# NoahVl/Explaining-In-Style-Reproducibility-Study

Measured on AMD Instinct MI355X. Metric: StylEx G+D+enc train-step images/sec @256px, higher is better.
Workload: dtype bf16; 1 GPU; FFHQ-shaped 256x256 StylEx, batch 32/GPU, GAE=2 (noise+encoder micro-steps), GP every 4th step, ResNet-18 classifier; image_size=256, batch_per_gpu=32, start_step=0, gradient_accumulate_every=2, global_batch=32, parallelism=dp1

## Files before the change

### explaining-in-style-reproducibility-study_amd/csrc/conv_halo_dma.hip

```cpp
#include <hip/hip_runtime.h>
#include <stdint.h>
#include <stdlib.h>

#include <type_traits>

#include "stylex_internal.h"

typedef float f32x16 __attribute__((ext_vector_type(16)));
typedef short bf16x8 __attribute__((ext_vector_type(8)));
typedef __bf16 bf16x2_t __attribute__((ext_vector_type(2)));
typedef float f32x2_t __attribute__((ext_vector_type(2)));

namespace {

__device__ uint4 g_zero_page_fwd[4];

typedef __attribute__((address_space(3))) void* lds_void_ptr;
typedef __attribute__((address_space(1))) const void* gl_void_ptr;

__device__ __forceinline__ unsigned short to_bf16(float v) {
    f32x2_t t = {v, 0.f};
    bf16x2_t r = __builtin_convertvector(t, bf16x2_t);
    return (unsigned short)(*reinterpret_cast<unsigned*>(&r) & 0xffffu);
}

constexpr int TW = 32, TH = 16, HWD = TW + 2, NP = (TH + 2) * HWD;
constexpr int ROW = 32;
constexpr int HALO_PIECES = (NP + 31) / 32;
constexpr int HALO_BYTES = HALO_PIECES * 1024;
template <int TNJ>
struct DmaCfg {
    static constexpr int BN = TNJ * 32;
    static constexpr int W_PIECES = 9 * BN / 32;
    static constexpr int PIECES = HALO_PIECES + W_PIECES;
    static constexpr int NIT = (PIECES + 3) / 4;
    static constexpr int BUF = PIECES * 1024;
    static constexpr int SMEM_BYTES = 2 * BUF;
};

template <int TNJ, unsigned MASK>
__device__ __forceinline__ void dma_chunk_masked(const char* base, const int (&a_off)[6][3], int b_lane,
                                                 f32x16 (&acc)[4][TNJ]) {
    constexpr int BN = TNJ * 32;
#pragma unroll
    for (int tap = 0; tap < 9; ++tap) {
        if (!((MASK >> tap) & 1u)) continue;
        const int kh = tap / 3, kw = tap - kh * 3;
        const int slot = __builtin_popcount(MASK & ((1u << tap) - 1u));
        bf16x8 av[4], bv[TNJ];
#pragma unroll
        for (int i = 0; i < 4; ++i) av[i] = *reinterpret_cast<const bf16x8*>(base + a_off[i + kh][kw]);
#pragma unroll
        for (int j = 0; j < TNJ; ++j)
            bv[j] = *reinterpret_cast<const bf16x8*>(base + b_lane + (slot * BN + j * 32) * ROW);
#pragma unroll
        for (int i = 0; i < 4; ++i)
#pragma unroll
            for (int j = 0; j < TNJ; ++j)
                acc[i][j] = __builtin_amdgcn_mfma_f32_32x32x16_bf16(bv[j], av[i], acc[i][j], 0, 0, 0);
    }
}

constexpr unsigned S2D_DGRAD_MASK[4] = {1u << 4, (1u << 4) | (1u << 5), (1u << 4) | (1u << 7),
                                        (1u << 4) | (1u << 5) | (1u << 7) | (1u << 8)};

constexpr unsigned S2D_FWD_MASK[4] = {1u << 4, (1u << 3) | (1u << 4), (1u << 1) | (1u << 4),
                                      (1u << 0) | (1u << 1) | (1u << 3) | (1u << 4)};
__device__ __forceinline__ int s2d_fwd_taps(int q) { return q == 0 ? 0x4 : q == 1 ? 0x43 : q == 2 ? 0x41 : 0x4310; }
__device__ __forceinline__ int s2d_fwd_ntaps(int q) { return q == 0 ? 1 : q == 3 ? 4 : 2; }

template <int TNJ, bool S2D = false>
__global__ __launch_bounds__(256, TNJ == 4 ? 1 : 2) void conv3x3_halo_dma_kernel(ConvKParams p) {
    constexpr int BN = DmaCfg<TNJ>::BN, PIECES = DmaCfg<TNJ>::PIECES, NIT = DmaCfg<TNJ>::NIT, BUF = DmaCfg<TNJ>::BUF;
    extern __shared__ __attribute__((aligned(16))) char smem[];
    const int tid = threadIdx.x, lane = tid & 63, wave = tid >> 6;
    const int H = p.Ho, W = p.Wo, C = p.Ck, N = p.N;
    const int n_tiles = (N + BN - 1) / BN;
    const int tiles_x = (W + TW - 1) / TW, tiles_y = (H + TH - 1) / TH;

    int bid = blockIdx.x;
    {
        int nblk = gridDim.x, q = nblk >> 3, rr = nblk & 7, xcd = bid & 7, idx = bid >> 3;
        bid = (xcd < rr ? xcd * (q + 1) : rr * (q + 1) + (xcd - rr) * q) + idx;
    }
    const int n0 = (bid % n_tiles) * BN;
    int pt = bid / n_tiles;
    const int b = pt / (tiles_x * tiles_y);
    pt -= b * tiles_x * tiles_y;
    const int y0 = (pt / tiles_x) * TH, x0 = (pt % tiles_x) * TW;

    const unsigned short* xs = reinterpret_cast<const unsigned short*>(p.a);
    const unsigned short* ws = reinterpret_cast<const unsigned short*>(p.w);
    const unsigned short* zero = reinterpret_cast<const unsigned short*>(g_zero_page_fwd);
    const int lr = lane >> 1, pslot = lane & 1;
    const int slot = pslot ^ ((lr >> 3) & 1);

    long src_off[NIT];
    bool src_ok[NIT];
    int wslot[NIT];
#pragma unroll
    for (int it = 0; it < NIT; ++it) {
        const int piece = wave + 4 * it;
        src_off[it] = 0;
        src_ok[it] = false;
        wslot[it] = 0;
        if (piece >= PIECES) continue;
        if (piece < HALO_PIECES) {
            const int hp = piece * 32 + lr;
            const int hh = hp / HWD, ww = hp - hh * HWD;
            const int y = y0 - 1 + hh, x = x0 - 1 + ww;
            src_ok[it] = hp < NP && y >= 0 && y < H && x >= 0 && x < W;
            src_off[it] = ((long)(b * H + y) * W + x) * C + slot * 8;
        } else {
            const int r = (piece - HALO_PIECES) * 32 + lr;
            int tap = r / BN;
            const int nl = r - tap * BN;
            bool tap_ok = true;
            wslot[it] = tap;
            if (S2D && !p.flip_taps) {
                tap = 0;
            } else if (S2D) {
                const unsigned m = S2D_DGRAD_MASK[n0 / p.s2d_c];
                tap_ok = tap < __builtin_popcount(m);
                unsigned mm = m;
// ... 104 lines not shown
        const bool more = ch + 1 < nchunks;
        const char* base = smem + buf * BUF;
#pragma unroll
        for (int tap = 0; tap < 9; ++tap) {
            const int kh = tap / 3, kw = tap - kh * 3;
            bf16x8 av[4], bv[TNJ];
#pragma unroll
            for (int i = 0; i < 4; ++i)
                av[i] = *reinterpret_cast<const bf16x8*>(base + a_off[i + kh][kw]);
#pragma unroll
            for (int j = 0; j < TNJ; ++j)
                bv[j] = *reinterpret_cast<const bf16x8*>(base + b_lane + (tap * BN + j * 32) * ROW);
#pragma unroll
            for (int i = 0; i < 4; ++i)
#pragma unroll
                for (int j = 0; j < TNJ; ++j)
                    acc[i][j] = __builtin_amdgcn_mfma_f32_32x32x16_bf16(bv[j], av[i], acc[i][j], 0, 0, 0);
            if (more && 2 * tap < NIT) {
                issue_piece((ch + 1) * 16, buf ^ 1, 2 * tap);
                if (2 * tap + 1 < NIT) issue_piece((ch + 1) * 16, buf ^ 1, 2 * tap + 1);
            }
        }
    }
    const int lj = lane & 31, lh = lane >> 5;
    const bool act = (p.flags & (STYLEX_EPI_LRELU | STYLEX_EPI_RELU)) != 0;
    const float slope = (p.flags & STYLEX_EPI_RELU) ? 0.f : 0.2f;
    unsigned short* yout = reinterpret_cast<unsigned short*>(p.y);
    const unsigned short* gate = (!S2D && (p.flags & STYLEX_EPI_GATE)) ? reinterpret_cast<const unsigned short*>(p.residual) : nullptr;
    const float gslope = p.res_scale;
    const unsigned char* gmask = S2D ? nullptr : p.gate_mask;
    unsigned char* mask_out = S2D ? nullptr : p.mask;
    auto gatem = [&](unsigned u, unsigned bits) -> unsigned {
        const float a0 = __uint_as_float(u << 16), c0 = __uint_as_float(u & 0xffff0000u);
        return (unsigned)to_bf16((bits & 1u) ? a0 : gslope * a0) | ((unsigned)to_bf16((bits & 2u) ? c0 : gslope * c0) << 16);
    };
    auto gate2 = [&](unsigned u, unsigned g) -> unsigned {
        const float a0 = __uint_as_float(u << 16), c0 = __uint_as_float(u & 0xffff0000u);
        const float ga = __uint_as_float(g << 16), gc = __uint_as_float(g & 0xffff0000u);
        return (unsigned)to_bf16(ga > 0.f ? a0 : gslope * a0) | ((unsigned)to_bf16(gc > 0.f ? c0 : gslope * c0) << 16);
    };
    {
        const unsigned short* res = (S2D && (p.flags & STYLEX_EPI_RESIDUAL)) ? reinterpret_cast<const unsigned short*>(p.residual) : nullptr;
        const float rsc = p.res_scale;
        const bool merged = S2D && !p.flip_taps && p.x2 != nullptr;
        float4 b4[TNJ][4];
#pragma unroll
        for (int j = 0; j < TNJ; ++j)
#pragma unroll
            for (int g = 0; g < 4; ++g) {
                const int n = n0 + j * 32 + 8 * g + 4 * lh;
                b4[j][g] = ((p.flags & STYLEX_EPI_BIAS) && n < N) ? *reinterpret_cast<const float4*>(p.bias + n)
                                                                  : make_float4(0.f, 0.f, 0.f, 0.f);
            }
#pragma unroll
        for (int i = 0; i < 4; ++i) {
            const int y = y0 + 4 * wave + i, x = x0 + lj;
            const bool pix_ok = y < H && x < W;
            const long obase = ((long)(b * H + y) * W + x) * N;
#pragma unroll
            for (int j = 0; j < TNJ; ++j) {
                unsigned P[4][2];
#pragma unroll
                for (int g = 0; g < 4; ++g) {
                    float v0 = acc[i][j][4 * g + 0] + b4[j][g].x, v1 = acc[i][j][4 * g + 1] + b4[j][g].y;
                    float v2 = acc[i][j][4 * g + 2] + b4[j][g].z, v3 = acc[i][j][4 * g + 3] + b4[j][g].w;
                    if (res) {
                        const int n = n0 + j * 32 + 8 * g + 4 * lh;
                        uint2 rv = make_uint2(0u, 0u);
                        if (pix_ok && n < N) rv = *reinterpret_cast<const uint2*>(res + obase + n);
                        v0 = (v0 + __uint_as_float(rv.x << 16)) * rsc;
                        v1 = (v1 + __uint_as_float(rv.x & 0xffff0000u)) * rsc;
                        v2 = (v2 + __uint_as_float(rv.y << 16)) * rsc;
                        v3 = (v3 + __uint_as_float(rv.y & 0xffff0000u)) * rsc;
                    } else if (merged) {
                        v0 *= rsc;
                        v1 *= rsc;
                        v2 *= rsc;
                        v3 *= rsc;
                    }
                    if (act) {
                        v0 = v0 > 0.f ? v0 : slope * v0;
                        v1 = v1 > 0.f ? v1 : slope * v1;
                        v2 = v2 > 0.f ? v2 : slope * v2;
                        v3 = v3 > 0.f ? v3 : slope * v3;
                    }
                    P[g][0] = (unsigned)to_bf16(v0) | ((unsigned)to_bf16(v1) << 16);
                    P[g][1] = (unsigned)to_bf16(v2) | ((unsigned)to_bf16(v3) << 16);
                }
#pragma unroll
                for (int g = 0; g < 4; g += 2)
#pragma unroll
                    for (int h = 0; h < 2; ++h) {
                        auto r = __builtin_amdgcn_permlane32_swap(P[g][h], P[g + 1][h], false, false);
                        P[g][h] = r[0];
                        P[g + 1][h] = r[1];
                    }
#pragma unroll
                for (int q = 0; q < 2; ++q) {
                    const int n = n0 + j * 32 + 16 * q + 8 * lh;
                    if (pix_ok && n < N) {
                        uint4 v = make_uint4(P[2 * q][0], P[2 * q][1], P[2 * q + 1][0], P[2 * q + 1][1]);
                        const long o = obase + n;
                        if (gate) {
                            const uint4 gv = *reinterpret_cast<const uint4*>(gate + o);
                            v.x = gate2(v.x, gv.x);
                            v.y = gate2(v.y, gv.y);
                            v.z = gate2(v.z, gv.z);
                            v.w = gate2(v.w, gv.w);
                        } else if (gmask) {
                            const unsigned m = gmask[o >> 3];
                            v.x = gatem(v.x, m);
                            v.y = gatem(v.y, m >> 2);
                            v.z = gatem(v.z, m >> 4);
                            v.w = gatem(v.w, m >> 6);
                        }
                        *reinterpret_cast<uint4*>(yout + o) = v;
                        if (mask_out) mask_out[o >> 3] = (unsigned char)stylex_sign_bits8(v);
                    }
                }
            }
        }
    }
}

}

template <int TNJ, bool S2D = false>
static int launch_dma(const ConvKParams& p, hipStream_t s) {
    static bool attr_done = false;
    if (!attr_done) {
        hipError_t e = hipFuncSetAttribute(reinterpret_cast<const void*>(conv3x3_halo_dma_kernel<TNJ, S2D>),
                                           hipFuncAttributeMaxDynamicSharedMemorySize, DmaCfg<TNJ>::SMEM_BYTES);
        if (e != hipSuccess) return (int)e;
        attr_done = true;
    }
    long tiles = (long)p.B * ((p.Wo + TW - 1) / TW) * ((p.Ho + TH - 1) / TH);
    long blocks = tiles * ((p.N + DmaCfg<TNJ>::BN - 1) / DmaCfg<TNJ>::BN);
    stylex_note_kernel("conv3x3_halo_dma_kernel<%d, %s>", TNJ, S2D ? "true" : "false");
    hipLaunchKernelGGL((conv3x3_halo_dma_kernel<TNJ, S2D>), dim3((unsigned)blocks), dim3(256), DmaCfg<TNJ>::SMEM_BYTES, s, p);
    return (int)hipGetLastError();
}

int stylex_launch_halo_dma(const ConvKParams& p, hipStream_t s) {
    static const bool on = !(getenv("STYLEX_HALO_DMA") && getenv("STYLEX_HALO_DMA")[0] == '0');
    static const bool on64 = !(getenv("STYLEX_HALO_DMA64") && getenv("STYLEX_HALO_DMA64")[0] == '0');
    static const bool on_s2d = !(getenv("STYLEX_HALO_DMA_S2D") && getenv("STYLEX_HALO_DMA_S2D")[0] == '0');
    if (!on) return STYLEX_NOT_APPLICABLE;
    if (!p.act_bf16 || p.a_scale) return STYLEX_NOT_APPLICABLE;
    if (p.flags & ~(STYLEX_EPI_BIAS | STYLEX_EPI_LRELU | STYLEX_EPI_RELU |
                    (p.s2d_c ? STYLEX_EPI_RESIDUAL : (STYLEX_EPI_GATE | STYLEX_EPI_GATE_MASK | STYLEX_EPI_MASK_OUT))))
        return STYLEX_NOT_APPLICABLE;
    if (p.s2d_c && (p.mask || p.gate_mask)) return STYLEX_NOT_APPLICABLE;
    if (p.x2) {
        if (!p.s2d_c || p.flip_taps || !p.w2 || p.c2 < 8 || p.c2 % 8 != 0 || (p.flags & STYLEX_EPI_RESIDUAL)) return STYLEX_NOT_APPLICABLE;
        if ((reinterpret_cast<uintptr_t>(p.x2) & 15) || (reinterpret_cast<uintptr_t>(p.w2) & 15)) return STYLEX_NOT_APPLICABLE;
    }
    if ((p.flags & STYLEX_EPI_GATE) && (!p.residual || (reinterpret_cast<uintptr_t>(p.residual) & 15))) return STYLEX_NOT_APPLICABLE;
    if (p.s2d_c && on_s2d) {
        const int rc = p.flip_taps ? stylex_launch_s2d_dgrad(p, s) : stylex_launch_s2d_fwd(p, s);
        if (rc != STYLEX_NOT_APPLICABLE) return rc;
    }
    if (p.N % 8 != 0 || p.Ck % 8 != 0 || p.Wo < 32 || p.Ho < 16) return STYLEX_NOT_APPLICABLE;
    if ((reinterpret_cast<uintptr_t>(p.a) & 15) || (reinterpret_cast<uintptr_t>(p.w) & 15) ||
        (reinterpret_cast<uintptr_t>(p.y) & 15))
        return STYLEX_NOT_APPLICABLE;
    if (p.s2d_c) {
        if (!on_s2d || !on64 || p.s2d_c % 64 != 0) return STYLEX_NOT_APPLICABLE;
        if (p.flip_taps) {
            if (p.flags || p.N != 4 * p.s2d_c || p.Ck < 64) return STYLEX_NOT_APPLICABLE;
        } else {
            static const bool on_fwd = !(getenv("STYLEX_HALO_DMA_S2D_FWD") && getenv("STYLEX_HALO_DMA_S2D_FWD")[0] == '0');
            if (!on_fwd || (p.flags & ~(STYLEX_EPI_BIAS | STYLEX_EPI_RESIDUAL)) || p.Ck != 4 * p.s2d_c || p.N % 64 != 0)
                return STYLEX_NOT_APPLICABLE;
            if ((p.flags & STYLEX_EPI_RESIDUAL) && (!p.residual || (reinterpret_cast<uintptr_t>(p.residual) & 15)))
                return STYLEX_NOT_APPLICABLE;
        }
        return p.dry ? 0 : launch_dma<2, true>(p, s);
    }
    if (on64 && p.Ck >= 64 && p.N % 64 == 0) return p.dry ? 0 : launch_dma<2>(p, s);
    static const bool on32 = !(getenv("STYLEX_HALO_DMA32") && getenv("STYLEX_HALO_DMA32")[0] == '0');
    if (on32 && on64 && p.Ck >= 64 && p.N <= 32) return p.dry ? 0 : launch_dma<1>(p, s);
    if (p.N >= 128 && p.Ck >= 128) return p.dry ? 0 : launch_dma<4>(p, s);
    return STYLEX_NOT_APPLICABLE;
}
```

### explaining-in-style-reproducibility-study_amd/csrc/conv_pipe.hip

```cpp
#include <hip/hip_runtime.h>
#include <stdint.h>
#include <stdlib.h>

#include "stylex_internal.h"

#ifndef PIPE_STORE_AUX
#define PIPE_STORE_AUX 0
#endif

typedef float f32x16 __attribute__((ext_vector_type(16)));
typedef short bf16x8 __attribute__((ext_vector_type(8)));
typedef __bf16 bf16x2_t __attribute__((ext_vector_type(2)));
typedef float f32x2_t __attribute__((ext_vector_type(2)));
typedef unsigned u32x4 __attribute__((ext_vector_type(4)));

struct StylexPipeArgs {
    int total_tiles;
    unsigned m_ntiles, m_tpi, m_tx;
    int dbg;
};

#ifdef STYLEX_PIPE_ABLATION
#define PIPE_DBG (pa.dbg)
#else
#define PIPE_DBG 0
#endif


namespace {

typedef StylexPipeArgs PipeArgs;
typedef __attribute__((address_space(3))) void* lds_void_ptr;

__device__ __forceinline__ unsigned short to_bf16(float v) {
    f32x2_t t = {v, 0.f};
    bf16x2_t r = __builtin_convertvector(t, bf16x2_t);
    return (unsigned short)(*reinterpret_cast<unsigned*>(&r) & 0xffffu);
}

template <int NT>
struct PipeCfg {
    static constexpr int TH = NT == 128 ? 16 : 32;
    static constexpr int TW = 32, HWD = TW + 2, NP = (TH + 2) * HWD;
    static constexpr int H_PIECES = (NP + 31) / 32;
    static constexpr int H_STRIDE = H_PIECES * 1024;
    static constexpr int W_PIECES = 9 * NT / 32;
    static constexpr int W_STRIDE = W_PIECES * 1024;
    static constexpr int HS = 3, WS = 2;
    static constexpr int W_BASE = HS * H_STRIDE;
    static constexpr int BIAS_BASE = W_BASE + WS * W_STRIDE;
    static constexpr int DUMP_BASE = BIAS_BASE + 2048;
    static constexpr int SMEM = DUMP_BASE + 1024;
    static constexpr int HP_MAX = (H_PIECES + 7) / 8;
    static constexpr int WP_MAX = (W_PIECES + 7) / 8;
    static constexpr int RG = TH / 4;
};

__device__ __forceinline__ void dma16(__amdgpu_buffer_rsrc_t r, char* smem, int lds_off, unsigned voff, unsigned soff) {
    __builtin_amdgcn_raw_ptr_buffer_load_lds(r, (lds_void_ptr)(smem + lds_off), 16, voff, soff, 0, 0);
}

template <int N>
__device__ __forceinline__ void wait_vmcnt() {
    asm volatile("s_waitcnt vmcnt(%0)" ::"n"(N) : "memory");
}

template <int OFF>
__device__ __forceinline__ void lds_read16(bf16x8& dst, int addr) {
    asm volatile("ds_read_b128 %0, %1 offset:%2" : "=v"(dst) : "v"(addr), "n"(OFF));
}
__device__ __forceinline__ void lds_wait(bf16x8 (&av)[4], bf16x8 (&bv)[2]) {
    asm volatile("s_waitcnt lgkmcnt(0)" : "+v"(av[0]), "+v"(av[1]), "+v"(av[2]), "+v"(av[3]), "+v"(bv[0]), "+v"(bv[1]));
}
template <int HWD, int TAP>
__device__ __forceinline__ void tap_addr(int (&addr)[4], int a_base, unsigned& swz) {
    constexpr int kh = TAP / 3, kw = TAP % 3;
    asm volatile("" : "+v"(swz));
#pragma unroll
    for (int i = 0; i < 4; ++i) addr[i] = a_base + ((i + kh) * HWD + kw) * 32 + (int)(((swz >> ((i + kh) * 3 + kw)) & 1u) << 4);
}
template <int NT, int TAP>
__device__ __forceinline__ void load_tap(bf16x8 (&av)[4], bf16x8 (&bv)[2], const int (&addr)[4], int b_addr) {
    lds_read16<(TAP * NT) * 32>(bv[0], b_addr);
    lds_read16<(TAP * NT + 32) * 32>(bv[1], b_addr);
#pragma unroll
    for (int i = 0; i < 4; ++i) lds_read16<0>(av[i], addr[i]);
}

__device__ __forceinline__ void mfma1(f32x16& acc, const bf16x8& a, const bf16x8& b) {
    asm volatile("v_mfma_f32_32x32x16_bf16 %0, %1, %2, %0" : "+v"(acc) : "v"(a), "v"(b));
}
__device__ __forceinline__ void mfma8(f32x16 (&acc)[4][2], const bf16x8 (&av)[4], const bf16x8 (&bv)[2]) {
#pragma unroll
    for (int i = 0; i < 4; ++i)
#pragma unroll
        for (int j = 0; j < 2; ++j) mfma1(acc[i][j], bv[j], av[i]);
}

__device__ __forceinline__ int fastdiv(int n, unsigned magic) { return magic ? (int)__umulhi((unsigned)n, magic) : n; }


template <int NT, int EPI>
__global__ __launch_bounds__(512, 2) void conv3x3_pipe_kernel(ConvKParams p, PipeArgs pa) {
    using Cfg = PipeCfg<NT>;
    constexpr int TH = Cfg::TH, HWD = Cfg::HWD, NP = Cfg::NP, H_PIECES = Cfg::H_PIECES, H_STRIDE = Cfg::H_STRIDE;
// ... 74 lines not shown
#pragma unroll
    for (int r = 0; r < 6; ++r)
#pragma unroll
        for (int kw = 0; kw < 3; ++kw) {
            const int t = a_row + r * HWD + kw;
            swz |= (unsigned)(((t >> 3) ^ lk) & 1) << (r * 3 + kw);
        }
    const int b_cur0 = W_BASE + (nh * 64 + li) * 32 + ((((li >> 3) ^ lk) & 1) << 4), b_cur1 = b_cur0 + W_STRIDE;

    if (EPI == 0 && (p.flags & STYLEX_EPI_BIAS) && tid < N) reinterpret_cast<float*>(smem + Cfg::BIAS_BASE)[tid] = p.bias[tid];

    f32x16 acc[4][2];
    auto zero_acc = [&]() {
#pragma unroll
        for (int i = 0; i < 4; ++i)
#pragma unroll
            for (int j = 0; j < 2; ++j)
#pragma unroll
                for (int e = 0; e < 16; ++e) acc[i][j][e] = 0.f;
    };
    zero_acc();

    const bool act = EPI == 0 && (p.flags & (STYLEX_EPI_LRELU | STYLEX_EPI_RELU)) != 0;
    const float slope = (p.flags & STYLEX_EPI_RELU) ? 0.f : 0.2f;
    const float gslope = p.res_scale;
    const bool mask_out = EPI == 0 && p.mask != nullptr;
    auto gatem = [&](unsigned u, unsigned bits) -> unsigned {
        const float a0 = __uint_as_float(u << 16), c0 = __uint_as_float(u & 0xffff0000u);
        f32x2_t t = {(bits & 1u) ? a0 : gslope * a0, (bits & 2u) ? c0 : gslope * c0};
        bf16x2_t r = __builtin_convertvector(t, bf16x2_t);
        return *reinterpret_cast<unsigned*>(&r);
    };
    auto gate2 = [&](unsigned u, unsigned g) -> unsigned {
        const float a0 = __uint_as_float(u << 16), c0 = __uint_as_float(u & 0xffff0000u);
        const float ga = __uint_as_float(g << 16), gc = __uint_as_float(g & 0xffff0000u);
        f32x2_t t = {ga > 0.f ? a0 : gslope * a0, gc > 0.f ? c0 : gslope * c0};
        bf16x2_t r = __builtin_convertvector(t, bf16x2_t);
        return *reinterpret_cast<unsigned*>(&r);
    };
    const unsigned bytes_y = (unsigned)((long)p.B * H * W * N * 2);
    const __amdgpu_buffer_rsrc_t ry = __builtin_amdgcn_make_buffer_rsrc(p.y, 0, (int)bytes_y, 0x00020000);
    const __amdgpu_buffer_rsrc_t rgate = __builtin_amdgcn_make_buffer_rsrc(const_cast<float*>(p.residual), 0, (int)bytes_y, 0x00020000);
    const __amdgpu_buffer_rsrc_t rmask = __builtin_amdgcn_make_buffer_rsrc(
        EPI == 2 ? const_cast<unsigned char*>(p.gate_mask) : p.mask, 0, (int)(bytes_y >> 4), 0x00020000);
    const unsigned rowb = (unsigned)(W * N) * 2u;
    auto pack2 = [](float a, float c) -> unsigned {
        f32x2_t t = {a, c};
        bf16x2_t r = __builtin_convertvector(t, bf16x2_t);
        return *reinterpret_cast<unsigned*>(&r);
    };
    const unsigned lane_off = (unsigned)(((4 * rg) * W + (lane & 7)) * N + nh * 64) * 2u +
                              (unsigned)(4 * ((lane >> 4) & 1) + 2 * ((lane >> 3) & 1) + (lane >> 5)) * 16u;
    const unsigned pixb8 = (unsigned)N * 16u;
    auto epilogue = [&](int b, int y0, int x0, int n0) {
        const int lh = lk;
        const int nb = n0 + nh * 64;
        const unsigned t_off = __builtin_amdgcn_readfirstlane((unsigned)((((long)(b * H + y0) * W + x0) * N + n0) * 2));
        const unsigned g_off = x0 + li < W ? (unsigned)(((4 * rg) * W + li) * N + nh * 64 + 8 * lh) * 2u : OOB;
#pragma unroll
        for (int i = 0; i < 4; ++i) {
            const bool row_ok = y0 + 4 * rg + i < H;
            const unsigned soff = t_off + i * rowb;
            u32x4 R[4];
#pragma unroll
            for (int j = 0; j < 2; ++j) {
                u32x4 gv[2];
                unsigned gm[2];
                if (EPI != 0) {
                    const unsigned voff = row_ok ? g_off : OOB;
#pragma unroll
                    for (int q = 0; q < 2; ++q) {
                        if (EPI == 1) gv[q] = __builtin_amdgcn_raw_buffer_load_b128(rgate, voff + (j * 64 + q * 32), soff, 0);
                        if (EPI == 2) gm[q] = __builtin_amdgcn_raw_buffer_load_b8(rmask, (voff >> 4) + (j * 4 + q * 2), soff >> 4, 0);
                    }
                }
                float4 b4[4];
#pragma unroll
                for (int g = 0; g < 4; ++g)
                    b4[g] = (EPI == 0 && (p.flags & STYLEX_EPI_BIAS))
                                ? *reinterpret_cast<const float4*>(smem + Cfg::BIAS_BASE + (nb + j * 32 + 8 * g + 4 * lh) * 4)
                                : make_float4(0.f, 0.f, 0.f, 0.f);
                unsigned P[4][2];
#pragma unroll
                for (int g = 0; g < 4; ++g) {
                    float v0 = acc[i][j][4 * g + 0] + b4[g].x, v1 = acc[i][j][4 * g + 1] + b4[g].y;
                    float v2 = acc[i][j][4 * g + 2] + b4[g].z, v3 = acc[i][j][4 * g + 3] + b4[g].w;
                    if (act) {
                        v0 = v0 > 0.f ? v0 : slope * v0;
                        v1 = v1 > 0.f ? v1 : slope * v1;
                        v2 = v2 > 0.f ? v2 : slope * v2;
                        v3 = v3 > 0.f ? v3 : slope * v3;
                    }
                    P[g][0] = pack2(v0, v1);
                    P[g][1] = pack2(v2, v3);
                }
#pragma unroll
                for (int g = 0; g < 4; g += 2)
#pragma unroll
                    for (int h = 0; h < 2; ++h) {
                        auto r = __builtin_amdgcn_permlane32_swap(P[g][h], P[g + 1][h], false, false);
                        P[g][h] = r[0];
                        P[g + 1][h] = r[1];
                    }
#pragma unroll
                for (int q = 0; q < 2; ++q) {
                    uint4 v = make_uint4(P[2 * q][0], P[2 * q][1], P[2 * q + 1][0], P[2 * q + 1][1]);
                    if (EPI == 1) {
                        v.x = gate2(v.x, gv[q].x);
                        v.y = gate2(v.y, gv[q].y);
                        v.z = gate2(v.z, gv[q].z);
                        v.w = gate2(v.w, gv[q].w);
                    } else if (EPI == 2) {
                        const unsigned m = gm[q];
                        v.x = gatem(v.x, m);
                        v.y = gatem(v.y, m >> 2);
                        v.z = gatem(v.z, m >> 4);
// ... 113 lines not shown
    __builtin_amdgcn_sched_barrier(0);
#define PIPE_CHUNK(A1, B1, A2, B2, BCUR, BNEXT, MORE_W, MORE_H)                                    \
    {                                                                                              \
        const bool mw_ = MORE_W, mh_ = MORE_H;                                                     \
        const unsigned w_soff = (unsigned)(w_n0 * 9 * C + w_ch * 16) * 2u, h_soff = (unsigned)h_ch * 32u; \
        PIPE_TAP(0, A1, B1, A2, B2, BCUR, mw_, mh_)                                                \
        PIPE_TAP(1, A2, B2, A1, B1, BCUR, mw_, mh_)                                                \
        PIPE_TAP(2, A1, B1, A2, B2, BCUR, mw_, mh_)                                                \
        PIPE_TAP(3, A2, B2, A1, B1, BCUR, mw_, mh_)                                                \
        PIPE_TAP(4, A1, B1, A2, B2, BCUR, mw_, mh_)                                                \
        PIPE_TAP(5, A2, B2, A1, B1, BCUR, mw_, mh_)                                                \
        PIPE_TAP(6, A1, B1, A2, B2, BCUR, mw_, mh_)                                                \
        PIPE_TAP(7, A2, B2, A1, B1, BCUR, mw_, mh_)                                                \
        PIPE_LAST(A1, B1, A2, B2, BNEXT)                                                           \
        if (mw_) adv_w();                                                                          \
        if (mh_) adv_h();                                                                          \
    }
    for (int g = 0; g < total; g += 2) {
        PIPE_CHUNK(avA, bvA, avB, bvB, b_cur0, b_cur1, g + 1 < total, g + 2 < total)
        PIPE_CHUNK(avB, bvB, avA, bvA, b_cur1, b_cur0, g + 2 < total, g + 3 < total)
        c_ch += 2;
        if (c_ch == nchunks) {
            c_ch = 0;
            asm volatile("s_nop 15\n\ts_nop 15"
                         : "+v"(acc[0][0]), "+v"(acc[0][1]), "+v"(acc[1][0]), "+v"(acc[1][1]), "+v"(acc[2][0]), "+v"(acc[2][1]),
                           "+v"(acc[3][0]), "+v"(acc[3][1]));
            epilogue(cb, cy0, cx0, cn0);
            if (++c_k < my_tiles) {
                decode(c_k, cb, cy0, cx0, cn0);
                zero_acc();
            }
        }
    }
#undef PIPE_CHUNK
#undef PIPE_LAST
#undef PIPE_TAP
#undef PIPE_DMA
#undef issue_h1
#undef issue_w1
    asm volatile("s_waitcnt lgkmcnt(0)" ::: "memory");
    wait_vmcnt<0>();
}

int g_num_cus = 0;

unsigned magic_of(int d) { return d <= 1 ? 0u : (unsigned)(((1ull << 32) + (unsigned)d - 1) / (unsigned)d); }

template <int NT, int EPI>
int launch_pipe(const ConvKParams& p, hipStream_t s) {
    using Cfg = PipeCfg<NT>;
    static bool attr_done = false;
    if (!attr_done) {
        hipError_t e = hipFuncSetAttribute(reinterpret_cast<const void*>(conv3x3_pipe_kernel<NT, EPI>),
                                           hipFuncAttributeMaxDynamicSharedMemorySize, Cfg::SMEM);
        if (e != hipSuccess) return (int)e;
        attr_done = true;
    }
    if (!g_num_cus) {
        int dev = 0, n = 0;
        (void)hipGetDevice(&dev);
        (void)hipDeviceGetAttribute(&n, hipDeviceAttributeMultiprocessorCount, dev);
        g_num_cus = n > 0 ? (n & ~7) : 256;
        if (g_num_cus < 8) g_num_cus = 8;
    }
    const int tiles_x = (p.Wo + 31) / 32, tiles_y = (p.Ho + Cfg::TH - 1) / Cfg::TH, n_tiles = p.N / NT;
    PipeArgs pa;
    pa.total_tiles = p.B * tiles_x * tiles_y * n_tiles;
    pa.m_ntiles = magic_of(n_tiles);
    pa.m_tpi = magic_of(tiles_x * tiles_y);
    pa.m_tx = magic_of(tiles_x);
#ifdef STYLEX_PIPE_ABLATION
    pa.dbg = getenv("STYLEX_PIPE_DBG") ? atoi(getenv("STYLEX_PIPE_DBG")) : 0;
#else
    pa.dbg = 0;
#endif
    stylex_note_kernel("conv3x3_pipe_kernel<%d, %d>", NT, EPI);
    hipLaunchKernelGGL((conv3x3_pipe_kernel<NT, EPI>), dim3((unsigned)g_num_cus), dim3(512), Cfg::SMEM, s, p, pa);
    return (int)hipGetLastError();
}

template <int NT>
int launch_pipe_epi(const ConvKParams& p, hipStream_t s) {
    if (p.flags & STYLEX_EPI_GATE) return launch_pipe<NT, 1>(p, s);
    if (p.flags & STYLEX_EPI_GATE_MASK) return launch_pipe<NT, 2>(p, s);
    return launch_pipe<NT, 0>(p, s);
}

}

int stylex_launch_pipe(const ConvKParams& p, hipStream_t s) {
    const char* env = getenv("STYLEX_CONV_PIPE");
    if (env && env[0] == '0') return STYLEX_NOT_APPLICABLE;
    if (!p.act_bf16 || p.a_scale || p.s2d_c) return STYLEX_NOT_APPLICABLE;
    if (p.flags & ~(STYLEX_EPI_BIAS | STYLEX_EPI_LRELU | STYLEX_EPI_RELU | STYLEX_EPI_GATE | STYLEX_EPI_GATE_MASK | STYLEX_EPI_MASK_OUT))
        return STYLEX_NOT_APPLICABLE;
    if ((p.flags & STYLEX_EPI_GATE) && (!p.residual || (reinterpret_cast<uintptr_t>(p.residual) & 15))) return STYLEX_NOT_APPLICABLE;
    if (p.Ck < 64 || p.Ck % 32 != 0 || p.N % 64 != 0 || p.N > 512 || p.Wo < 32 || p.Ho < 16) return STYLEX_NOT_APPLICABLE;
    if ((reinterpret_cast<uintptr_t>(p.a) & 15) || (reinterpret_cast<uintptr_t>(p.w) & 15) || (reinterpret_cast<uintptr_t>(p.y) & 15))
        return STYLEX_NOT_APPLICABLE;
    if ((long)p.B * p.Ho * p.Wo * p.Ck * 2 >= (1l << 31) || (long)p.N * 9 * p.Ck * 2 >= (1l << 31) ||
        (long)p.B * p.Ho * p.Wo * p.N * 2 >= (1l << 31))
        return STYLEX_NOT_APPLICABLE;
    const bool n128 = p.N % 128 == 0 && !(env && env[0] == '6');
    if (!n128) {
        if (p.Ho < 32 && !(env && env[0] == '6')) return STYLEX_NOT_APPLICABLE;
        if (!(env && env[0] == '6') && ((p.flags & STYLEX_EPI_GATE) || (p.flip_taps && !p.flags && p.Ck == 64)))
            return STYLEX_NOT_APPLICABLE;
    }
    if (p.dry) return 0;
    if (n128) return launch_pipe_epi<128>(p, s);
    return launch_pipe_epi<64>(p, s);
}
```

### explaining-in-style-reproducibility-study_amd/csrc/elementwise.hip

```cpp
#include <hip/hip_runtime.h>
#include <stdint.h>

#include "stylex_internal.h"

namespace {

template <int V>
struct Vec;
template <>
struct Vec<4> {
    typedef float4 T;
    static __device__ __forceinline__ T zero() { return make_float4(0.f, 0.f, 0.f, 0.f); }
    static __device__ __forceinline__ T ld(const void* p, long off, int bf) { return act_ld4(p, off, bf); }
    static __device__ __forceinline__ void st(void* p, long off, T v, int bf) { act_st4(p, off, v, bf); }
    static __device__ __forceinline__ void fma(T& a, float w, T x) {
        a.x = fmaf(w, x.x, a.x); a.y = fmaf(w, x.y, a.y); a.z = fmaf(w, x.z, a.z); a.w = fmaf(w, x.w, a.w);
    }
};
template <>
struct Vec<1> {
    typedef float T;
    static __device__ __forceinline__ T zero() { return 0.f; }
    static __device__ __forceinline__ T ld(const void* p, long off, int bf) { return act_ld1(p, off, bf); }
    static __device__ __forceinline__ void st(void* p, long off, T v, int bf) { act_st1(p, off, v, bf); }
    static __device__ __forceinline__ void fma(T& a, float w, T x) { a = fmaf(w, x, a); }
};

struct F8 {
    float4 a, b;
};
template <>
struct Vec<8> {
    typedef F8 T;
    static __device__ __forceinline__ T zero() { return F8{make_float4(0.f, 0.f, 0.f, 0.f), make_float4(0.f, 0.f, 0.f, 0.f)}; }
    static __device__ __forceinline__ T ld(const void* p, long off, int) {
        uint4 h = *reinterpret_cast<const uint4*>(reinterpret_cast<const unsigned short*>(p) + off);
        return F8{act_unpack4(make_uint2(h.x, h.y)), act_unpack4(make_uint2(h.z, h.w))};
    }
    static __device__ __forceinline__ void st(void* p, long off, T v, int) {
        uint2 lo = act_pack4(v.a), hi = act_pack4(v.b);
        *reinterpret_cast<uint4*>(reinterpret_cast<unsigned short*>(p) + off) = make_uint4(lo.x, lo.y, hi.x, hi.y);
    }
    static __device__ __forceinline__ void fma(T& acc, float w, T x) {
        Vec<4>::fma(acc.a, w, x.a);
        Vec<4>::fma(acc.b, w, x.b);
    }
};

__device__ __forceinline__ void up_rule(int o, int n, int& lo, int& hi, float& w_hi) {
    int k = o >> 1;
    if (o & 1) {
        lo = k;
        hi = min(k + 1, n - 1);
        w_hi = 0.25f;
    } else {
        lo = max(k - 1, 0);
        hi = k;
        w_hi = 0.75f;
    }
}
__device__ __forceinline__ float up_coef(int o, int i, int n) {
    int lo, hi;
    float wh;
    up_rule(o, n, lo, hi, wh);
    return (lo == i ? 1.f - wh : 0.f) + (hi == i ? wh : 0.f);
}

__device__ __forceinline__ long decomp_index(long i, int cv, int Wd, int Hd, int& cq, int& w, int& h, int& b) {
    if (i < (1L << 31)) {
        const unsigned u = (unsigned)i, pix = u / (unsigned)cv, r = pix / (unsigned)Wd;
        cq = (int)(u - pix * (unsigned)cv);
        w = (int)(pix - r * (unsigned)Wd);
        b = (int)(r / (unsigned)Hd);
        h = (int)(r - (unsigned)b * (unsigned)Hd);
        return (long)pix;
    }
    const long pix = i / cv, r = pix / Wd;
    cq = (int)(i - pix * cv);
    w = (int)(pix - r * Wd);
    b = (int)(r / Hd);
    h = (int)(r - (long)b * Hd);
    return pix;
}

template <int V>
__global__ void upsample2x_fwd_kernel(const void* __restrict__ x, void* __restrict__ y, int B, int H, int W, int C, int bf) {
    const int cv = C / V;
    const long total = (long)B * 2 * H * 2 * W * cv;
    for (long i = blockIdx.x * (long)blockDim.x + threadIdx.x; i < total; i += (long)gridDim.x * blockDim.x) {
        int cq, ow, oh, b;
        const long pix = decomp_index(i, cv, (2 * W), (2 * H), cq, ow, oh, b);
        const int c = cq * V;
        int hl, hh, wl, wh_;
        float fh, fw;
        up_rule(oh, H, hl, hh, fh);
        up_rule(ow, W, wl, wh_, fw);
        const long base = (long)b * H * W * C + c;
        typename Vec<V>::T acc = Vec<V>::zero();
        typename Vec<V>::T r0 = Vec<V>::zero(), r1 = Vec<V>::zero();
        Vec<V>::fma(r0, 1.f - fw, Vec<V>::ld(x, base + ((long)hl * W + wl) * C, bf));
        Vec<V>::fma(r0, fw, Vec<V>::ld(x, base + ((long)hl * W + wh_) * C, bf));
        Vec<V>::fma(r1, 1.f - fw, Vec<V>::ld(x, base + ((long)hh * W + wl) * C, bf));
        Vec<V>::fma(r1, fw, Vec<V>::ld(x, base + ((long)hh * W + wh_) * C, bf));
        Vec<V>::fma(acc, 1.f - fh, r0);
        Vec<V>::fma(acc, fh, r1);
        Vec<V>::st(y, pix * C + c, acc, bf);
    }
}

template <int V>
__global__ void upsample2x_bwd_kernel(const void* __restrict__ dy, void* __restrict__ dx, int B, int H, int W, int C, int bf) {
    const int cv = C / V;
    const long total = (long)B * H * W * cv;
    for (long i = blockIdx.x * (long)blockDim.x + threadIdx.x; i < total; i += (long)gridDim.x * blockDim.x) {
        int cq, iw, ih, b;
        const long pix = decomp_index(i, cv, W, H, cq, iw, ih, b);
        const int c = cq * V;
        const long base = (long)b * 4 * H * W * C + c;
        typename Vec<V>::T acc = Vec<V>::zero();
#pragma unroll
        for (int a = -1; a <= 2; ++a) {
            int oh = 2 * ih + a;
            if (oh < 0 || oh >= 2 * H) continue;
            float ch = up_coef(oh, ih, H);
            if (ch == 0.f) continue;
#pragma unroll
            for (int e = -1; e <= 2; ++e) {
                int ow = 2 * iw + e;
                if (ow < 0 || ow >= 2 * W) continue;
                float cw = up_coef(ow, iw, W);
                if (cw == 0.f) continue;
                Vec<V>::fma(acc, ch * cw, Vec<V>::ld(dy, base + ((long)oh * 2 * W + ow) * C, bf));
            }
        }
        Vec<V>::st(dx, pix * C + c, acc, bf);
    }
}

__device__ __forceinline__ int reflect1(int i, int n) { return i < 0 ? -i : (i >= n ? 2 * n - 2 - i : i); }

__device__ __forceinline__ float ub_coef(int o, int i, int n) {
    const int n2 = 2 * n;
    return 0.25f * up_coef(reflect1(o - 1, n2), i, n) + 0.5f * up_coef(o, i, n) + 0.25f * up_coef(reflect1(o + 1, n2), i, n);
}

template <int V>
__global__ void rgb_up_blur_add_fwd_kernel(const void* __restrict__ rgb, const void* __restrict__ prev, void* __restrict__ y,
                                           int B, int H, int W, int C, int bf) {
    const int cv = C / V;
    const long total = (long)B * 2 * H * 2 * W * cv;
    for (long i = blockIdx.x * (long)blockDim.x + threadIdx.x; i < total; i += (long)gridDim.x * blockDim.x) {
        int cq, ow, oh, b;
        const long pix = decomp_index(i, cv, 2 * W, 2 * H, cq, ow, oh, b);
        const int c = cq * V, kh = oh >> 1, kw = ow >> 1;
        const long base = (long)b * H * W * C + c;
        float cw[3];
#pragma unroll
        for (int e = 0; e < 3; ++e) {
            const int iw = kw - 1 + e;
            cw[e] = (iw >= 0 && iw < W) ? ub_coef(ow, iw, W) : 0.f;
        }
        typename Vec<V>::T acc = Vec<V>::zero();
// ... 326 lines not shown
    long b = (work + 255) / 256;
    if (b > 2048) b = 2048;
    if (b < 1) b = 1;
    return (int)b;
}
inline bool vec_ok(int C, const void* a, const void* b) {
    return (C % 4 == 0) && ((reinterpret_cast<uintptr_t>(a) & 15) == 0) && ((reinterpret_cast<uintptr_t>(b) & 15) == 0);
}

}

#define LAUNCH_EW(kern, work, a, b, ...)                                                                    \
    do {                                                                                                    \
        if (bf && (C % 8 == 0) && vec_ok(C, a, b))                                                          \
            hipLaunchKernelGGL(kern<8>, dim3(grid_for((work) / 8)), dim3(256), 0, s, __VA_ARGS__);          \
        else if (vec_ok(C, a, b))                                                                           \
            hipLaunchKernelGGL(kern<4>, dim3(grid_for((work) / 4)), dim3(256), 0, s, __VA_ARGS__);          \
        else                                                                                                \
            hipLaunchKernelGGL(kern<1>, dim3(grid_for(work)), dim3(256), 0, s, __VA_ARGS__);                \
        return (int)hipGetLastError();                                                                      \
    } while (0)

static bool blur_strip_ok(int bf, int H, int C, const void* a, const void* b) {
    return bf && (C % 8 == 0) && H >= 8 && ((reinterpret_cast<uintptr_t>(a) & 15) == 0) &&
           ((reinterpret_cast<uintptr_t>(b) & 15) == 0);
}
template <bool ADJ>
static int launch_blur_strip(const void* in, void* out, int B, int H, int W, int C, int s2d, hipStream_t s,
                             const void* gate = nullptr, float gslope = 0.f, const void* gmask = nullptr) {
    constexpr int ROWS = 8;
    long work = (long)B * ((H + ROWS - 1) / ROWS) * W * (C / 8);
    long blocks = (work + 255) / 256;
    if (blocks > 16384) blocks = 16384;
    hipLaunchKernelGGL((blur3x3_strip_kernel<ADJ, ROWS>), dim3((unsigned)blocks), dim3(256), 0, s,
                       (const unsigned short*)in, (unsigned short*)out, B, H, W, C, s2d, (const unsigned short*)gate,
                       gslope, (const unsigned char*)gmask);
    return (int)hipGetLastError();
}

extern "C" {

#define EW_ARGS const int64_t* sh, int act_dtype, void* stream
#define EW_UNPACK                                                     \
    hipStream_t s = (hipStream_t)stream;                               \
    int B = (int)sh[0], H = (int)sh[1], W = (int)sh[2], C = (int)sh[3]; \
    int bf = act_dtype == 1;                                           \
    if (act_dtype != 0 && act_dtype != 1) return STYLEX_EINVAL;

int stylex_upsample2x_bilinear_fwd(const void* x, void* y, EW_ARGS) {
    EW_UNPACK
    if (B <= 0 || H <= 0 || W <= 0 || C <= 0) return STYLEX_EINVAL;
    LAUNCH_EW(upsample2x_fwd_kernel, (long)B * 4 * H * W * C, x, y, x, y, B, H, W, C, bf);
}
int stylex_upsample2x_bilinear_bwd(const void* dy, void* dx, EW_ARGS) {
    EW_UNPACK
    if (B <= 0 || H <= 0 || W <= 0 || C <= 0) return STYLEX_EINVAL;
    LAUNCH_EW(upsample2x_bwd_kernel, (long)B * H * W * C, dy, dx, dy, dx, B, H, W, C, bf);
}
int stylex_rgb_up_blur_add_fwd(const void* rgb, const void* prev, void* y, EW_ARGS) {
    EW_UNPACK
    if (!rgb || !y || B <= 0 || H <= 0 || W <= 0 || C <= 0) return STYLEX_EINVAL;
    const void* al = prev ? prev : rgb;
    if (vec_ok(C, rgb, y) && vec_ok(C, al, y))
        hipLaunchKernelGGL(rgb_up_blur_add_fwd_kernel<4>, dim3(grid_for((long)B * 4 * H * W * C / 4)), dim3(256), 0, s, rgb, prev,
                           y, B, H, W, C, bf);
    else
        hipLaunchKernelGGL(rgb_up_blur_add_fwd_kernel<1>, dim3(grid_for((long)B * 4 * H * W * C)), dim3(256), 0, s, rgb, prev, y,
                           B, H, W, C, bf);
    return (int)hipGetLastError();
}
int stylex_rgb_up_blur_add_bwd(const void* dy, void* dx, EW_ARGS) {
    EW_UNPACK
    if (!dy || !dx || B <= 0 || H <= 0 || W <= 0 || C <= 0) return STYLEX_EINVAL;
    LAUNCH_EW(rgb_up_blur_add_bwd_kernel, (long)B * H * W * C, dy, dx, dy, dx, B, H, W, C, bf);
}
int stylex_blur3x3_reflect_fwd(const void* x, void* y, EW_ARGS) {
    EW_UNPACK
    if (B <= 0 || H < 2 || W < 2 || C <= 0) return STYLEX_EINVAL;
    if (blur_strip_ok(bf, H, C, x, y)) return launch_blur_strip<false>(x, y, B, H, W, C, 0, s);
    LAUNCH_EW(blur3x3_fwd_kernel, (long)B * H * W * C, x, y, x, y, B, H, W, C, bf, 0);
}
static int blur_bwd_impl(const void* dy, const void* gate, float gslope, void* dx, int s2d, EW_ARGS) {
    EW_UNPACK
    if (B <= 0 || H < 2 || W < 2 || C <= 0 || (s2d && ((H & 1) || (W & 1)))) return STYLEX_EINVAL;
    const bool gate_ok = !gate || (reinterpret_cast<uintptr_t>(gate) & 15) == 0;
    if (gate_ok && blur_strip_ok(bf, H, C, dy, dx)) return launch_blur_strip<true>(dy, dx, B, H, W, C, s2d, s, gate, gslope);
    if (gate && !gate_ok) {
        hipLaunchKernelGGL(blur3x3_bwd_kernel<1>, dim3(grid_for((long)B * H * W * C)), dim3(256), 0, s, dy, dx, B, H, W, C, bf,
                           s2d, gate, gslope);
        return (int)hipGetLastError();
    }
    LAUNCH_EW(blur3x3_bwd_kernel, (long)B * H * W * C, dy, dx, dy, dx, B, H, W, C, bf, s2d, gate, gslope);
}
int stylex_blur3x3_reflect_bwd(const void* dy, void* dx, EW_ARGS) { return blur_bwd_impl(dy, nullptr, 0.f, dx, 0, sh, act_dtype, stream); }
int stylex_blur3x3_reflect_bwd_gate(const void* dy, const void* gate, float slope, void* dx, EW_ARGS) {
    if (!gate) return STYLEX_EINVAL;
    return blur_bwd_impl(dy, gate, slope, dx, 0, sh, act_dtype, stream);
}
int stylex_blur3x3_s2d_bwd_gate(const void* dy, const void* gate, float slope, void* dx, EW_ARGS) {
    if (!gate) return STYLEX_EINVAL;
    return blur_bwd_impl(dy, gate, slope, dx, 1, sh, act_dtype, stream);
}
int stylex_blur3x3_s2d_bwd_gate_mask(const void* dy, const void* mask, float slope, void* dx, EW_ARGS) {
    EW_UNPACK
    if (!dy || !mask || !dx || B <= 0 || H < 2 || W < 2 || C <= 0 || (H & 1) || (W & 1)) return STYLEX_EINVAL;
    if (!blur_strip_ok(bf, H, C, dy, dx)) return STYLEX_EINVAL;
// ... 82 lines not shown
```

### explaining-in-style-reproducibility-study_amd/csrc/fused_bwd.hip

```cpp
#include <hip/hip_runtime.h>
#include <stdint.h>

#include "stylex_internal.h"

namespace {

constexpr int NT = 256;

template <int K>
struct Acc {
    float4 v[K];
    __device__ __forceinline__ void zero() {
#pragma unroll
        for (int k = 0; k < K; ++k) v[k] = make_float4(0.f, 0.f, 0.f, 0.f);
    }
};

template <int K>
__device__ __forceinline__ void block_reduce_store(Acc<K>& a, float* smem, int cv, int prow, int CV, int rpp, int C,
                                                   float* partial_row , bool active) {
    float4* s4 = reinterpret_cast<float4*>(smem);
    if (active) {
#pragma unroll
        for (int k = 0; k < K; ++k) s4[(k * rpp + prow) * CV + cv] = a.v[k];
// ... 100 lines not shown
            float4 yv = ld4(y, o, bf);
            float nz = 0.f;
            if (noise) {
                const int pi = (int)p, h = pi / W, w = pi - h * W;
                nz = noise[((long)g.b * ns + w) * ns + h];
            }
            float4 t = yv;
            if (lrelu) {
                gv.x = yv.x > 0.f ? gv.x : 0.2f * gv.x; t.x = yv.x > 0.f ? yv.x : 5.f * yv.x;
                gv.y = yv.y > 0.f ? gv.y : 0.2f * gv.y; t.y = yv.y > 0.f ? yv.y : 5.f * yv.y;
                gv.z = yv.z > 0.f ? gv.z : 0.2f * gv.z; t.z = yv.z > 0.f ? yv.z : 5.f * yv.z;
                gv.w = yv.w > 0.f ? gv.w : 0.2f * gv.w; t.w = yv.w > 0.f ? yv.w : 5.f * yv.w;
            }
            if (gz_scale) st4(gz, o, make_float4(gv.x * d4.x, gv.y * d4.y, gv.z * d4.z, gv.w * d4.w), bf);
            else st4(gz, o, gv, bf);
            a.v[0].x += gv.x * (t.x - (nz * w4.x + b4.x));
            a.v[0].y += gv.y * (t.y - (nz * w4.y + b4.y));
            a.v[0].z += gv.z * (t.z - (nz * w4.z + b4.z));
            a.v[0].w += gv.w * (t.w - (nz * w4.w + b4.w));
            a.v[1].x += gv.x * nz; a.v[1].y += gv.y * nz; a.v[1].z += gv.z * nz; a.v[1].w += gv.w * nz;
            a.v[2].x += gv.x; a.v[2].y += gv.y; a.v[2].z += gv.z; a.v[2].w += gv.w;
        }
    }
    block_reduce_store<3>(a, smem, g.cv, g.prow, g.CV, g.rpp, C, partial + ((long)g.b * nchunks + blockIdx.x) * 3 * C,
                          g.active && c < C);
}

__global__ __launch_bounds__(NT) void scale_reduce_kernel(const void* __restrict__ x, const void* __restrict__ t,
                                                         const float* __restrict__ s, void* __restrict__ gx,
                                                         float* __restrict__ partial, int HW, int C, int nchunks, int bf) {
    extern __shared__ __attribute__((aligned(16))) float smem[];
    Geo g = make_geo(HW, C, nchunks);
    Acc<1> a;
    a.zero();
    const int c = g.cv * 4;
    if (g.active && c < C) {
        float4 s4 = ldp4(s + (long)g.b * C + c);
        const long base = (long)g.b * HW;
        for (long p = g.p_begin + g.prow; p < g.p_end; p += g.rpp) {
            const long o = (base + p) * C + c;
            float4 tv = ld4(t, o, bf);
            float4 xv = ld4(x, o, bf);
            a.v[0].x += xv.x * tv.x; a.v[0].y += xv.y * tv.y; a.v[0].z += xv.z * tv.z; a.v[0].w += xv.w * tv.w;
            if (gx) {
                tv.x *= s4.x; tv.y *= s4.y; tv.z *= s4.z; tv.w *= s4.w;
                st4(gx, o, tv, bf);
            }
        }
    }
    block_reduce_store<1>(a, smem, g.cv, g.prow, g.CV, g.rpp, C, partial + ((long)g.b * nchunks + blockIdx.x) * C,
                          g.active && c < C);
}

inline size_t reduce_smem(int C, int K) {
    int CV = (C + 3) / 4;
    if (CV > NT) CV = NT;
    int rpp = NT / CV;
    return (size_t)K * rpp * CV * 16;
}

inline bool ok_shape(const int64_t* sh, int nchunks) {
    return sh[0] > 0 && sh[1] > 0 && sh[2] > 0 && sh[3] > 0 && sh[3] <= 1024 && (sh[3] % 4 == 0) && nchunks > 0 &&
           sh[0] <= 65535;
}

}

extern "C" {

int stylex_reduce_chunks(const int64_t* sh) {
    long HW = (long)sh[1] * sh[2];
    long n = (2048 + sh[0] - 1) / sh[0];
    long maxc = (HW + 63) / 64;
    if (n > maxc) n = maxc;
    if (n < 1) n = 1;
    return (int)n;
}

int stylex_act_bwd_reduce(const void* dy, const void* y, void* dx, float* partial, const int64_t* sh, int nchunks,
                          int lrelu, float scale, int act_dtype, void* stream) {
    if (act_dtype != 0 && act_dtype != 1) return STYLEX_EINVAL;
    if (!dy || !partial || !ok_shape(sh, nchunks) || (lrelu && !y)) return STYLEX_EINVAL;
    int HW = (int)(sh[1] * sh[2]), C = (int)sh[3];
    hipLaunchKernelGGL(act_bwd_reduce_kernel, dim3(nchunks, (unsigned)sh[0]), dim3(NT), reduce_smem(C, 1),
                       (hipStream_t)stream, dy, y, dx, partial, HW, C, nchunks, lrelu, scale, act_dtype);
    return (int)hipGetLastError();
}

static int modconv_bwd_prep_impl(const void* gy, const void* y, const float* noise, int64_t noise_stride,
                                 const float* noise_w, const float* noise_b, void* gz, float* partial, const int64_t* sh,
                                 int nchunks, int lrelu, int act_dtype, const float* gz_scale, void* stream);

int stylex_modconv_bwd_prep(const void* gy, const void* y, const float* noise, int64_t noise_stride,
                            const float* noise_w, const float* noise_b, void* gz, float* partial, const int64_t* sh,
                            int nchunks, int lrelu, int act_dtype, void* stream) {
    return modconv_bwd_prep_impl(gy, y, noise, noise_stride, noise_w, noise_b, gz, partial, sh, nchunks, lrelu, act_dtype,
                                 nullptr, stream);
}

int stylex_modconv_bwd_prep_scaled(const void* gy, const void* y, const float* noise, int64_t noise_stride,
                                   const float* noise_w, const float* noise_b, const float* gz_scale, void* gz,
                                   float* partial, const int64_t* sh, int nchunks, int lrelu, int act_dtype, void* stream) {
    if (!gz_scale || (reinterpret_cast<uintptr_t>(gz_scale) & 15)) return STYLEX_EINVAL;
    return modconv_bwd_prep_impl(gy, y, noise, noise_stride, noise_w, noise_b, gz, partial, sh, nchunks, lrelu, act_dtype,
                                 gz_scale, stream);
}

static int modconv_bwd_prep_impl(const void* gy, const void* y, const float* noise, int64_t noise_stride,
                                 const float* noise_w, const float* noise_b, void* gz, float* partial, const int64_t* sh,
                                 int nchunks, int lrelu, int act_dtype, const float* gz_scale, void* stream) {
    if (act_dtype != 0 && act_dtype != 1) return STYLEX_EINVAL;
    if (!gy || !y || !gz || !partial || !ok_shape(sh, nchunks)) return STYLEX_EINVAL;
    if (noise && (!noise_w || !noise_b || noise_stride < sh[1] || noise_stride < sh[2])) return STYLEX_EINVAL;
    int C = (int)sh[3];
    hipLaunchKernelGGL(modconv_bwd_prep_kernel, dim3(nchunks, (unsigned)sh[0]), dim3(NT), reduce_smem(C, 3),
                       (hipStream_t)stream, gy, y, noise, (int)noise_stride, noise_w, noise_b, gz, partial, (int)sh[1],
                       (int)sh[2], C, nchunks, lrelu, act_dtype, gz_scale);
    return (int)hipGetLastError();
}

int stylex_scale_reduce(const void* x, const void* t, const float* s, void* gx, float* partial, const int64_t* sh,
                        int nchunks, int act_dtype, void* stream) {
    if (act_dtype != 0 && act_dtype != 1) return STYLEX_EINVAL;
    if (!x || !t || !s || !partial || !ok_shape(sh, nchunks)) return STYLEX_EINVAL;
    int HW = (int)(sh[1] * sh[2]), C = (int)sh[3];
    hipLaunchKernelGGL(scale_reduce_kernel, dim3(nchunks, (unsigned)sh[0]), dim3(NT), reduce_smem(C, 1),
                       (hipStream_t)stream, x, t, s, gx, partial, HW, C, nchunks, act_dtype);
    return (int)hipGetLastError();
}

}
```

### explaining-in-style-reproducibility-study_amd/csrc/stylex_capi.hip

```cpp
#include <hip/hip_runtime.h>
#include <stdint.h>
#include <stdarg.h>
#include <stdio.h>
#include <string.h>

#include <array>
#include <map>
#include <mutex>
#include <string>
#include <vector>

#include "stylex_internal.h"

namespace {

typedef std::array<int64_t, 9> LayerKey;
struct TimedLaunch {
    hipEvent_t start, stop;
    int cls;
    double flops;
    double bytes;
    LayerKey key;
    char kernel[112];
};
// ... 202 lines not shown
static void bwd_data_params(ConvKParams& p, const int64_t* sh) {
    fill_common(p, sh);
    p.Hi = (int)sh[9];
    p.Wi = (int)sh[10];
    p.Ck = (int)sh[4];
    p.N = (int)sh[3];
    p.Ho = (int)sh[1];
    p.Wo = (int)sh[2];
    p.M = p.B * p.Ho * p.Wo;
}

int64_t stylex_conv2d_workspace_bytes(const int64_t* sh, int which, int precision) {
    if (!conv_shape_ok(sh) || (which != 0 && which != 1)) return STYLEX_EINVAL;
    ConvKParams p;
    if (which == 0) fwd_params(p, sh);
    else {
        bwd_data_params(p, sh);
        p.transposed = 1;
    }
    p.act_bf16 = precision == STYLEX_BF16_ACT;
    return stylex_igemm_workspace_bytes(p, precision);
}

int stylex_conv_mask_supported(const int64_t* sh, int which, int flags, int precision) {
    if (!conv_shape_ok(sh) || precision != STYLEX_BF16_ACT || (which != 0 && which != 1)) return 0;
    static const uintptr_t fake = 4096;
    ConvKParams p;
    if (which == 0) {
        if (!(flags & STYLEX_EPI_MASK_OUT) || !(flags & STYLEX_EPI_LRELU)) return 0;
        fwd_params(p, sh);
        if (p.N % 8 != 0) return 0;
        p.mask = (unsigned char*)fake;
    } else {
        if (!(flags & STYLEX_EPI_GATE_MASK) || (flags & ~(STYLEX_EPI_GATE_MASK))) return 0;
        bwd_data_params(p, sh);
        if (p.KH != 3 || p.stride != 1 || p.pad != 1) return 0;
        p.flip_taps = 1;
        p.gate_mask = (const unsigned char*)fake;
    }
    p.a = (const float*)fake;
    p.w = (const void*)fake;
    p.y = (float*)fake;
    p.bias = (const float*)fake;
    p.flags = flags;
    p.act_bf16 = 1;
    p.dry = 1;
    if (which == 0 && stylex_launch_rgb(p, nullptr) == 0) return 1;
    return stylex_launch_halo(p, nullptr) == 0 ? 1 : 0;
}

int stylex_conv2d_fwd(const void* x, const void* w_fwd, void* y, const int64_t* sh, int flags,
                      const stylex_conv_epilogue* epi, int precision, void* workspace, int64_t workspace_bytes,
                      void* stream) {
    if (!x || !w_fwd || !y || !conv_shape_ok(sh)) return STYLEX_EINVAL;
    if (precision != STYLEX_F32 && precision != STYLEX_BF16 && precision != STYLEX_BF16_ACT) return STYLEX_EINVAL;
    ConvKParams p;
    fwd_params(p, sh);
    p.a = (const float*)x;
    p.w = w_fwd;
    p.y = (float*)y;
    p.flags = flags;
    p.act_bf16 = precision == STYLEX_BF16_ACT;
    if (p.act_bf16) precision = STYLEX_BF16;
    if (epi) {
        p.a_scale = epi->in_scale;
        p.bias = epi->bias;
        p.out_scale = epi->out_scale;
        p.noise = epi->noise;
        p.noise_stride = (int)epi->noise_stride;
        p.noise_w = epi->noise_w;
        p.noise_b = epi->noise_b;
        p.residual = (const float*)epi->residual;
        p.res_scale = epi->res_scale;
        p.s2d_c = (int)epi->s2d_c;
    }
    if (flags & STYLEX_EPI_GATE_MASK) return STYLEX_EINVAL;
    if (flags & STYLEX_EPI_MASK_OUT) {
        if (!epi || !epi->mask || !(flags & STYLEX_EPI_LRELU) || !p.act_bf16 || p.N % 8 != 0) return STYLEX_EINVAL;
        p.mask = (unsigned char*)epi->mask;
    }
    if ((flags & STYLEX_EPI_BIAS) && !p.bias) return STYLEX_EINVAL;
    if ((flags & STYLEX_EPI_OSCALE) && !p.out_scale) return STYLEX_EINVAL;
    if ((flags & STYLEX_EPI_NOISE_NAT) && (!(flags & STYLEX_EPI_NOISE) || (reinterpret_cast<uintptr_t>(p.noise) & 15) ||
                                           p.noise_stride % 4 != 0))
        return STYLEX_EINVAL;
    if ((flags & STYLEX_EPI_NOISE) && (!p.noise || !p.noise_w || !p.noise_b || p.noise_stride < p.Ho || p.noise_stride < p.Wo))
        return STYLEX_EINVAL;
    if ((flags & STYLEX_EPI_RESIDUAL) && !p.residual) return STYLEX_EINVAL;
    if (p.s2d_c && (p.Ck != 4 * p.s2d_c || p.KH != 3 || p.stride != 1 || p.pad != 1 || p.s2d_c % 64)) return STYLEX_EINVAL;
    double flops = 2.0 * p.M * (double)p.N * p.Ck * p.KH * p.KW / (p.s2d_c ? 4.0 : 1.0);
    ScopedTimer tm(0, flops, conv_bytes(sh, p.act_bf16 ? STYLEX_BF16_ACT : precision, false), (hipStream_t)stream, sh, p.s2d_c);
    return stylex_launch_igemm(p, precision, workspace, workspace_bytes, (hipStream_t)stream);
}

static int s2d_res_params(ConvKParams& p, const int64_t* sh, int64_t s2d_c, int64_t res_c) {
    if (!conv_shape_ok(sh)) return STYLEX_EINVAL;
    fwd_params(p, sh);
    p.s2d_c = (int)s2d_c;
    p.c2 = (int)res_c;
    if (s2d_c <= 0 || s2d_c % 64 || p.Ck != 4 * p.s2d_c || p.KH != 3 || p.stride != 1 || p.pad != 1) return STYLEX_EINVAL;
    if (res_c < 8 || res_c % 8) return STYLEX_EINVAL;
    p.act_bf16 = 1;
    p.flags = STYLEX_EPI_BIAS;
    return 0;
}

int stylex_conv2d_s2d_res_supported(const int64_t* sh, int64_t s2d_c, int64_t res_c) {
    static const uintptr_t fake = 4096;
    ConvKParams p;
    if (s2d_res_params(p, sh, s2d_c, res_c)) return 0;
    p.a = (const float*)fake;
    p.w = (const void*)fake;
    p.y = (float*)fake;
    p.bias = (const float*)fake;
    p.x2 = p.w2 = (const void*)fake;
    p.dry = 1;
    return stylex_launch_halo_dma(p, nullptr) == 0 ? 1 : 0;
}

int stylex_conv2d_s2d_res_fwd(const void* x_s2d, const void* w_fwd_s2d, const void* x_res, const void* w_res, const float* bias,
                              void* y, const int64_t* sh, int64_t s2d_c, int64_t res_c, float scale, void* stream) {
    if (!x_s2d || !w_fwd_s2d || !x_res || !w_res || !bias || !y) return STYLEX_EINVAL;
    ConvKParams p;
    if (int rc = s2d_res_params(p, sh, s2d_c, res_c)) return rc;
    p.a = (const float*)x_s2d;
    p.w = w_fwd_s2d;
    p.y = (float*)y;
    p.bias = bias;
    p.x2 = x_res;
    p.w2 = w_res;
    p.res_scale = scale;
    const double flops = 2.0 * p.M * (double)p.N * (p.Ck * 9 / 4.0 + p.c2);
    ScopedTimer tm(0, flops, conv_bytes(sh, STYLEX_BF16_ACT, false) + 2.0 * p.M * p.c2, (hipStream_t)stream, sh, p.s2d_c);
    const int rc = stylex_launch_halo_dma(p, (hipStream_t)stream);
    return rc == STYLEX_NOT_APPLICABLE ? STYLEX_EINVAL : rc;
}

int stylex_conv2d_bwd_data(const void* dy, const void* w_bwd, void* dx, const int64_t* sh, int flags,
                           const stylex_conv_epilogue* epi, int precision, void* workspace, int64_t workspace_bytes,
                           void* stream) {
    if (!dy || !w_bwd || !dx || !conv_shape_ok(sh) || sh[7] > 2) return STYLEX_EINVAL;
    if (precision != STYLEX_F32 && precision != STYLEX_BF16 && precision != STYLEX_BF16_ACT) return STYLEX_EINVAL;
    if (flags & ~(STYLEX_EPI_OSCALE | STYLEX_EPI_GATE | STYLEX_EPI_GATE_MASK)) return STYLEX_EINVAL;
    if ((flags & STYLEX_EPI_GATE) && (!epi || !epi->residual)) return STYLEX_EINVAL;
// ... 173 lines not shown
```

### explaining-in-style-reproducibility-study_amd/csrc/stylex_internal.h

```cpp
#pragma once
#include <hip/hip_runtime.h>
#include <stdint.h>

#include "../../include/stylex_hip.h"
#include "act_io.h"

struct ConvKParams {
    const float* a;
    const float* a_scale;
    const void* w;
    const float* a2;
    const float* a2_scale;
    float* y;
    const float* bias;
    const float* out_scale;
    const float* noise;
    const float* noise_w;
    const float* noise_b;
    const float* residual;
    float res_scale;
    int noise_stride;
    int B, Hi, Wi, Ck, N, KH, KW, Ho, Wo, stride, pad;
    int transposed;
    int phase_major;
    int act_bf16;
    int s2d_c;
    int flip_taps;
    int M;
    int flags;
    long split_len;
    int ksplit;
    int kt_per_split;
    float* partial;
    unsigned char* mask;
    const unsigned char* gate_mask;
    int dry;
    float* bias_partial;
    const void* x2;
    const void* w2;
    int c2;
    float wg_scale;
    int wg_accumulate;
};

int stylex_launch_igemm(ConvKParams p, int precision, void* workspace, int64_t workspace_bytes, hipStream_t s);
int64_t stylex_igemm_workspace_bytes(const ConvKParams& p, int precision);
void stylex_wgrad_plan(const ConvKParams& p, int* tn, int* tc, int* splits, long* split_len);
int stylex_launch_wgrad(ConvKParams p, float* partial, float* dw_oihw, int precision, hipStream_t s, float* db = nullptr,
                        int* db_done = nullptr);
int stylex_launch_pack(const float* w, void* wf, void* wb, int N, int C, int T, int dtype, hipStream_t s);

#define STYLEX_NOT_APPLICABLE (-100)

void stylex_note_kernel(const char* fmt, ...);

#ifdef __HIPCC__
__device__ __forceinline__ unsigned stylex_sign_bits8(uint4 v) {
    const unsigned w[4] = {v.x, v.y, v.z, v.w};
    unsigned m = 0;
#pragma unroll
    for (int d = 0; d < 4; ++d) {
        m |= (__uint_as_float(w[d] << 16) > 0.f ? 1u : 0u) << (2 * d);
        m |= (__uint_as_float(w[d] & 0xffff0000u) > 0.f ? 1u : 0u) << (2 * d + 1);
    }
    return m;
}
#endif
int stylex_launch_halo(const ConvKParams& p, hipStream_t s);

int stylex_launch_halo_dma(const ConvKParams& p, hipStream_t s);

int stylex_launch_rgb(const ConvKParams& p, hipStream_t s);

int stylex_launch_pipe(const ConvKParams& p, hipStream_t s);
int stylex_launch_line64(const ConvKParams& p, hipStream_t s);

int stylex_launch_s2d_dgrad(const ConvKParams& p, hipStream_t s);
int stylex_launch_s2d_fwd(const ConvKParams& p, hipStream_t s);

int stylex_launch_gather(ConvKParams& p, void* workspace, int64_t workspace_bytes, hipStream_t s);
int64_t stylex_gather_workspace_bytes(const ConvKParams& p);

bool stylex_wgrad_pipe_applicable(const ConvKParams& p);
void stylex_wgrad_pipe_plan(const ConvKParams& p, int* slices, int* tiles_per_split, int* blocks);
int stylex_launch_wgrad_pipe(ConvKParams p, float* partial, hipStream_t s, int* slices_out, int* bias_done = nullptr);
int stylex_launch_wgrad_s2d_folded(ConvKParams p, float* partial, float* dw_oihw, hipStream_t s);

bool stylex_wgrad_tr_applicable(const ConvKParams& p);
void stylex_wgrad_tr_plan(const ConvKParams& p, int* mode, int* splits, long* split_len);
int stylex_launch_wgrad_tr(ConvKParams p, float* partial, hipStream_t s, int* splits_out);

__host__ __device__ inline unsigned stylex_s2d_tap_mask(int s) {
    const int sy = s >> 1, sx = s & 1;
    unsigned m = 0;
    for (int kh = 0; kh < 2; ++kh)
        for (int kw = 0; kw < 2; ++kw)
            if ((kh == 1 || sy == 1) && (kw == 1 || sx == 1)) m |= 1u << (kh * 3 + kw);
    return m;
}
int stylex_launch_pack_s2d(const float* w, void* wf, void* wb, int N, int C, hipStream_t s);
int stylex_launch_fold_s2d(const float* dw2, float* dw, int N, int C, hipStream_t s);
```

### explaining-in-style-reproducibility-study_amd/stylex/hip_backend.py

```python
import os as _os

if _os.environ.get("STYLEX_MIOPEN_ALLOW_BWD_GTC", "0") != "1":
    _os.environ.setdefault("MIOPEN_DEBUG_CONV_IMPLICIT_GEMM_ASM_BWD_GTC_XDLOPS_NHWC", "0")

import atexit
import ctypes
import os
import weakref

import torch

_HERE = os.path.dirname(os.path.abspath(__file__))
LIB_PATH = os.path.join(os.path.dirname(_HERE), "libstylex_hip.so")

F32, BF16, BF16_ACT = 0, 1, 2
EPI_BIAS, EPI_LRELU, EPI_OSCALE, EPI_NOISE, EPI_RESIDUAL, EPI_RELU, EPI_GATE, EPI_NOISE_NAT = 1, 2, 4, 8, 16, 32, 64, 128
EPI_MASK_OUT, EPI_GATE_MASK = 256, 512

_c_f = ctypes.c_void_p
_i64p = ctypes.POINTER(ctypes.c_int64)


class ConvEpilogue(ctypes.Structure):
    _fields_ = [
        ("in_scale", ctypes.c_void_p),
        ("bias", ctypes.c_void_p),
        ("out_scale", ctypes.c_void_p),
        ("noise", ctypes.c_void_p),
        ("noise_stride", ctypes.c_int64),
        ("noise_w", ctypes.c_void_p),
        ("noise_b", ctypes.c_void_p),
        ("residual", ctypes.c_void_p),
        ("res_scale", ctypes.c_float),
        ("s2d_c", ctypes.c_int32),
        ("mask", ctypes.c_void_p),
    ]


SIGNATURES = {
    "stylex_init": (ctypes.c_int, [ctypes.c_int]),
    "stylex_version": (ctypes.c_char_p, []),
    "stylex_pack_weight": (ctypes.c_int, [_c_f, _c_f, _c_f, _i64p, ctypes.c_int, ctypes.c_void_p]),
    "stylex_conv2d_workspace_bytes": (ctypes.c_int64, [_i64p, ctypes.c_int, ctypes.c_int]),
    "stylex_conv2d_fwd": (ctypes.c_int, [_c_f, _c_f, _c_f, _i64p, ctypes.c_int, ctypes.POINTER(ConvEpilogue),
                                         ctypes.c_int, ctypes.c_void_p, ctypes.c_int64, ctypes.c_void_p]),
    "stylex_conv2d_bwd_data": (ctypes.c_int, [_c_f, _c_f, _c_f, _i64p, ctypes.c_int, ctypes.POINTER(ConvEpilogue),
                                              ctypes.c_int, ctypes.c_void_p, ctypes.c_int64, ctypes.c_void_p]),
    "stylex_conv2d_bwd_weight_workspace_bytes": (ctypes.c_int64, [_i64p]),
    "stylex_conv2d_bwd_weight": (ctypes.c_int, [_c_f, _c_f, _c_f, ctypes.c_void_p, ctypes.c_int64, _i64p, _c_f, _c_f,
                                                ctypes.c_int, ctypes.c_int, ctypes.c_void_p]),
    "stylex_conv2d_bwd_weight_bias": (ctypes.c_int, [_c_f, _c_f, _c_f, _c_f, ctypes.POINTER(ctypes.c_int), ctypes.c_void_p,
                                                     ctypes.c_int64, _i64p, _c_f, _c_f, ctypes.c_int, ctypes.c_int,
                                                     ctypes.c_void_p]),
    "stylex_conv2d_bwd_weight_ex": (ctypes.c_int, [_c_f, _c_f, _c_f, _c_f, ctypes.POINTER(ctypes.c_int), ctypes.c_void_p,
                                                   ctypes.c_int64, _i64p, _c_f, _c_f, ctypes.c_int, ctypes.c_float, ctypes.c_int,
                                                   ctypes.c_int, ctypes.c_void_p]),
    "stylex_blur3x3_s2d_fwd": (ctypes.c_int, [_c_f, _c_f, _i64p, ctypes.c_int, ctypes.c_void_p]),
    "stylex_blur3x3_s2d_bwd": (ctypes.c_int, [_c_f, _c_f, _i64p, ctypes.c_int, ctypes.c_void_p]),
    "stylex_blur3x3_reflect_bwd_gate": (ctypes.c_int, [_c_f, _c_f, ctypes.c_float, _c_f, _i64p, ctypes.c_int, ctypes.c_void_p]),
    "stylex_blur3x3_s2d_bwd_gate": (ctypes.c_int, [_c_f, _c_f, ctypes.c_float, _c_f, _i64p, ctypes.c_int, ctypes.c_void_p]),
    "stylex_blur3x3_s2d_bwd_gate_mask": (ctypes.c_int, [_c_f, _c_f, ctypes.c_float, _c_f, _i64p, ctypes.c_int, ctypes.c_void_p]),
    "stylex_conv_mask_supported": (ctypes.c_int, [_i64p, ctypes.c_int, ctypes.c_int, ctypes.c_int]),
    "stylex_add_at_even": (ctypes.c_int, [_c_f, _c_f, _i64p, ctypes.c_int, ctypes.c_void_p]),
    "stylex_subsample2_fwd": (ctypes.c_int, [_c_f, _c_f, _i64p, ctypes.c_int, ctypes.c_void_p]),
    "stylex_subsample2_bwd": (ctypes.c_int, [_c_f, _c_f, _i64p, ctypes.c_int, ctypes.c_void_p]),
    "stylex_pack_weight_s2d": (ctypes.c_int, [_c_f, _c_f, _c_f, _i64p, ctypes.c_void_p]),
    "stylex_fold_weight_grad_s2d": (ctypes.c_int, [_c_f, _c_f, _i64p, ctypes.c_void_p]),
    "stylex_conv2d_bwd_weight_s2d_supported": (ctypes.c_int, [_i64p, ctypes.c_int, ctypes.c_int]),
    "stylex_conv2d_bwd_weight_s2d": (ctypes.c_int, [ctypes.c_void_p, ctypes.c_void_p, _c_f, ctypes.c_void_p, ctypes.c_int64, _i64p,
                                                    ctypes.c_int, ctypes.c_float, ctypes.c_int, ctypes.c_int, ctypes.c_void_p]),
    "stylex_upsample2x_bilinear_fwd": (ctypes.c_int, [_c_f, _c_f, _i64p, ctypes.c_int, ctypes.c_void_p]),
    "stylex_upsample2x_bilinear_bwd": (ctypes.c_int, [_c_f, _c_f, _i64p, ctypes.c_int, ctypes.c_void_p]),
    "stylex_rgb_up_blur_add_fwd": (ctypes.c_int, [_c_f, _c_f, _c_f, _i64p, ctypes.c_int, ctypes.c_void_p]),
    "stylex_rgb_up_blur_add_bwd": (ctypes.c_int, [_c_f, _c_f, _i64p, ctypes.c_int, ctypes.c_void_p]),
    "stylex_blur3x3_reflect_fwd": (ctypes.c_int, [_c_f, _c_f, _i64p, ctypes.c_int, ctypes.c_void_p]),
    "stylex_blur3x3_reflect_bwd": (ctypes.c_int, [_c_f, _c_f, _i64p, ctypes.c_int, ctypes.c_void_p]),
    "stylex_bias_act_fwd": (ctypes.c_int, [_c_f, _c_f, _c_f, ctypes.c_int64, _c_f, _c_f, _c_f, _i64p, ctypes.c_int,
                                           ctypes.c_void_p]),
    "stylex_bias_act_bwd": (ctypes.c_int, [_c_f, _c_f, _c_f, _i64p, ctypes.c_int, ctypes.c_void_p]),
    "stylex_rowwise_sumsq": (ctypes.c_int, [_c_f, _c_f, _i64p, ctypes.c_void_p]),
    "stylex_reduce_chunks": (ctypes.c_int, [_i64p]),
    "stylex_act_bwd_reduce": (ctypes.c_int, [_c_f, _c_f, _c_f, _c_f, _i64p, ctypes.c_int, ctypes.c_int, ctypes.c_float,
                                             ctypes.c_int, ctypes.c_void_p]),
    "stylex_modconv_bwd_prep": (ctypes.c_int, [_c_f, _c_f, _c_f, ctypes.c_int64, _c_f, _c_f, _c_f, _c_f, _i64p,
                                               ctypes.c_int, ctypes.c_int, ctypes.c_int, ctypes.c_void_p]),
    "stylex_modconv_bwd_prep_scaled": (ctypes.c_int, [_c_f, _c_f, _c_f, ctypes.c_int64, _c_f, _c_f, _c_f, _c_f, _c_f, _i64p,
                                                      ctypes.c_int, ctypes.c_int, ctypes.c_int, ctypes.c_void_p]),
    "stylex_scale_reduce": (ctypes.c_int, [_c_f, _c_f, _c_f, _c_f, _c_f, _i64p, ctypes.c_int, ctypes.c_int,
                                           ctypes.c_void_p]),
    "stylex_pad_rgb8": (ctypes.c_int, [_c_f, _c_f, _i64p, _i64p, ctypes.c_int, ctypes.c_void_p]),
    "stylex_affine_act_nchw_fwd": (ctypes.c_int, [_c_f, _c_f, _c_f, _c_f, _c_f, ctypes.c_int64, ctypes.c_int64, ctypes.c_int64,
                                                  ctypes.c_int, ctypes.c_void_p]),
    "stylex_affine_act_nchw_bwd": (ctypes.c_int, [_c_f, _c_f, _c_f, _c_f, _c_f, ctypes.c_int64, ctypes.c_int64, ctypes.c_int64,
                                                  ctypes.c_int, ctypes.c_void_p]),
    "stylex_affine_relu_maxpool_fwd": (ctypes.c_int, [_c_f, _c_f, _c_f, _c_f, _c_f, ctypes.c_int64, ctypes.c_int64,
                                                      ctypes.c_int64, ctypes.c_int64, ctypes.c_void_p]),
    "stylex_affine_relu_maxpool_bwd": (ctypes.c_int, [_c_f, _c_f, _c_f, _c_f, ctypes.c_int64, ctypes.c_int64, ctypes.c_int64,
                                                      ctypes.c_int64, ctypes.c_void_p]),
    "stylex_lpips_tap_nhwc_fwd": (ctypes.c_int, [_c_f, _c_f, _c_f, _c_f, _c_f, _c_f, ctypes.c_int64, ctypes.c_int64, ctypes.c_int64,
                                                 ctypes.c_int64, ctypes.c_void_p]),
    "stylex_lpips_tap_nhwc_bwd": (ctypes.c_int, [_c_f, _c_f, _c_f, _c_f, _c_f, _c_f, _c_f, _c_f, ctypes.c_int64, ctypes.c_int64,
                                                 ctypes.c_int64, ctypes.c_void_p]),
    "stylex_nchw_f32_to_nhwc_bf16": (ctypes.c_int, [_c_f, _c_f, ctypes.c_int64, ctypes.c_int64, ctypes.c_int64, ctypes.c_int,
                                                    ctypes.c_void_p]),
    "stylex_nhwc_bf16_to_nchw_f32": (ctypes.c_int, [_c_f, _c_f, _c_f, ctypes.c_int64, ctypes.c_int64, ctypes.c_int64, ctypes.c_void_p]),
    "stylex_resize_norm_fwd": (ctypes.c_int, [_c_f, _c_f, _c_f, _c_f, _i64p, _i64p, ctypes.c_void_p]),
    "stylex_resize_norm_bwd": (ctypes.c_int, [_c_f, _c_f, _c_f, _i64p, ctypes.c_void_p]),
    "stylex_relu_gate_add": (ctypes.c_int, [_c_f, _c_f, _c_f, _c_f, ctypes.c_int64, ctypes.c_void_p]),
    "stylex_maxpool3s2_nhwc_fwd": (ctypes.c_int, [_c_f, _c_f, _c_f, _i64p, ctypes.c_void_p]),
    "stylex_maxpool3s2_nhwc_bwd": (ctypes.c_int, [_c_f, _c_f, _c_f, _i64p, ctypes.c_void_p]),
    "stylex_conv_image_grad": (ctypes.c_int, [_c_f, _c_f, _c_f, _i64p, ctypes.c_void_p]),
    "stylex_lpips_tap_fwd": (ctypes.c_int, [_c_f, _c_f, _c_f, _c_f, _c_f, _c_f, ctypes.c_int64, ctypes.c_int64, ctypes.c_int64,
                                            ctypes.c_int64, ctypes.c_void_p]),
    "stylex_lpips_tap_bwd": (ctypes.c_int, [_c_f, _c_f, _c_f, _c_f, _c_f, _c_f, _c_f, _c_f, ctypes.c_int64, ctypes.c_int64,
                                            ctypes.c_int64, ctypes.c_void_p]),
    "stylex_weight_sumsq": (ctypes.c_int, [_c_f, _c_f, ctypes.c_int64, ctypes.c_int64, ctypes.c_int64, ctypes.c_void_p]),
    "stylex_modcoeff_fwd": (ctypes.c_int, [_c_f, _c_f, _c_f, _c_f, ctypes.c_int64, ctypes.c_int64, ctypes.c_int64,
                                           ctypes.c_float, ctypes.c_void_p]),
    "stylex_modcoeff_bwd": (ctypes.c_int, [_c_f, _c_f, _c_f, _c_f, _c_f, _c_f, _c_f, _c_f, ctypes.c_int64, ctypes.c_int64,
                                           ctypes.c_int64, ctypes.c_int64, ctypes.c_void_p]),
    "stylex_torgb_chunks": (ctypes.c_int, [_i64p]),
    "stylex_torgb_fwd": (ctypes.c_int, [_c_f, _c_f, _c_f, _c_f, _i64p, ctypes.c_void_p]),
    "stylex_torgb_bwd": (ctypes.c_int, [_c_f, _c_f, _c_f, _c_f, _c_f, _c_f, _i64p, ctypes.c_void_p]),
    "stylex_timing_enable": (ctypes.c_int, [ctypes.c_int]),
    "stylex_timing_pause": (ctypes.c_int, [ctypes.c_int]),
    "stylex_timing_layers": (ctypes.c_int, [_i64p, ctypes.POINTER(ctypes.c_double), ctypes.c_int64]),
    "stylex_timing_kernels": (ctypes.c_int, [ctypes.c_char_p, _i64p, ctypes.POINTER(ctypes.c_double), ctypes.c_int64]),
    "stylex_conv2d_s2d_res_supported": (ctypes.c_int, [_i64p, ctypes.c_int64, ctypes.c_int64]),
    "stylex_conv2d_s2d_res_fwd": (ctypes.c_int, [ctypes.c_void_p] * 6 + [_i64p, ctypes.c_int64, ctypes.c_int64, ctypes.c_float,
                                                  ctypes.c_void_p]),
    "stylex_adam_pack_tensor_blocks": (ctypes.c_int64, [ctypes.c_int64, ctypes.c_int32, ctypes.c_int32, ctypes.c_int32]),
    "stylex_adam_pack_step": (ctypes.c_int, [ctypes.c_void_p, ctypes.c_void_p, ctypes.c_int64, ctypes.c_void_p]),
    "stylex_hinge_fwd": (ctypes.c_int, [_c_f, _c_f, _c_f, ctypes.c_int64, ctypes.c_int, ctypes.c_void_p]),
    "stylex_hinge_bwd": (ctypes.c_int, [_c_f] * 5 + [ctypes.c_int64, ctypes.c_int, ctypes.c_void_p]),
    "stylex_pl_lengths_fwd": (ctypes.c_int, [_c_f, _c_f, _i64p, ctypes.c_void_p]),
    "stylex_pl_lengths_bwd": (ctypes.c_int, [_c_f] * 4 + [_i64p, ctypes.c_void_p]),
    "stylex_kl_logits_fwd": (ctypes.c_int, [_c_f, _c_f, _c_f, _i64p, ctypes.c_void_p]),
    "stylex_kl_logits_bwd": (ctypes.c_int, [_c_f] * 5 + [_i64p, ctypes.c_void_p]),
    "stylex_l1_mean_chunks": (ctypes.c_int64, [ctypes.c_int64]),
    "stylex_l1_mean_fwd": (ctypes.c_int, [_c_f] * 4 + [ctypes.c_int64, ctypes.c_int, ctypes.c_int, _i64p, _i64p, _i64p,
                                            ctypes.c_void_p]),
    "stylex_l1_mean_bwd": (ctypes.c_int, [_c_f] * 5 + [ctypes.c_int64, ctypes.c_int, ctypes.c_int, _i64p, _i64p, _i64p,
# ... 594 lines not shown
def fold_weight_grad_s2d(dw2, w_shape):
    lib = _ensure_device(dw2)
    n, c = w_shape[0], w_shape[1]
    dw = _empty(tuple(w_shape), dtype=torch.float32, device=dw2.device)
    _check(lib.stylex_fold_weight_grad_s2d(_ptr(dw2.contiguous()), _ptr(dw), _shape(n, c, 3, 3), _stream()),
           "stylex_fold_weight_grad_s2d")
    return dw


def _split_workspace(lib, shp, which, precision, like):
    nbytes = lib.stylex_conv2d_workspace_bytes(shp, which, precision)
    if nbytes <= 0:
        return None, 0
    return _empty(nbytes // 4, dtype=torch.float32, device=like.device), nbytes


_MASK_OK = {}


def conv_mask_supported(sh, which, flags, precision):
    key = (tuple(sh), which, flags, precision)
    hit = _MASK_OK.get(key)
    if hit is None:
        hit = _MASK_OK[key] = bool(load_library().stylex_conv_mask_supported(_shape(*sh), which, flags, precision))
    return hit


_S2D_RES_OK = {}


def s2d_res_supported(xb_shape, n, s2d_c, res_c):
    key = (tuple(xb_shape), n, s2d_c, res_c)
    hit = _S2D_RES_OK.get(key)
    if hit is None:
        sh = conv_shape(xb_shape, (n, xb_shape[1], 3, 3), 1, 1)
        hit = _S2D_RES_OK[key] = bool(load_library().stylex_conv2d_s2d_res_supported(_shape(*sh), s2d_c, res_c))
    return hit


def conv2d_s2d_res_fwd(xb, wf2, xs, w_res_mat, bias, n, s2d_c, scale):
    lib = _ensure_device(xb)
    assert is_cl(xb) and is_cl(xs) and xb.dtype == torch.bfloat16 and xs.dtype == torch.bfloat16
    assert xs.shape[0] == xb.shape[0] and xs.shape[2:] == xb.shape[2:] and w_res_mat.shape == (n, xs.shape[1])
    sh = conv_shape(xb.shape, (n, xb.shape[1], 3, 3), 1, 1)
    y = empty_cl((sh[0], n, sh[9], sh[10]), xb, torch.bfloat16)
    bias = _f32(bias)
    _check(lib.stylex_conv2d_s2d_res_fwd(_ptr(xb), _ptr(wf2), _ptr(xs), _ptr(w_res_mat), _ptr(bias), _ptr(y), _shape(*sh),
                                         int(s2d_c), int(xs.shape[1]), float(scale), _stream()), "stylex_conv2d_s2d_res_fwd")
    return y


def conv2d_fwd(x, w, stride, pad, precision, bias=None, lrelu=False, in_scale=None, out_scale=None, noise=None,
               noise_w=None, noise_b=None, residual=None, res_scale=1.0, packed=None, w_shape=None, s2d_c=0,
               noise_natural=False, want_mask=False):
    lib = _ensure_device(x)
    adt = act_dtype(precision)
    assert is_cl(x) and x.dtype == adt, (x.dtype, adt)
    sh = conv_shape(x.shape, w_shape if packed is not None else w.shape, stride, pad)
    wf = packed if packed is not None else pack_weight(w, True, False, precision)[0]
    y = empty_cl((sh[0], sh[4], sh[9], sh[10]), x, adt)
    flags = 0
    epi = ConvEpilogue()
    epi.s2d_c = int(s2d_c)
    keep = []
    if in_scale is not None:
        in_scale = _f32(in_scale)
        keep.append(in_scale)
        epi.in_scale = in_scale.data_ptr()
    if bias is not None:
        bias = _f32(bias)
        keep.append(bias)
        flags |= EPI_BIAS
        epi.bias = bias.data_ptr()
    if lrelu:
        flags |= EPI_RELU if lrelu == "relu" else EPI_LRELU
    if out_scale is not None:
        out_scale = _f32(out_scale)
        keep.append(out_scale)
        flags |= EPI_OSCALE
        epi.out_scale = out_scale.data_ptr()
    if noise is not None:
        noise, noise_w, noise_b = _f32(noise), _f32(noise_w), _f32(noise_b)
        keep += [noise, noise_w, noise_b]
        flags |= EPI_NOISE | (EPI_NOISE_NAT if noise_natural else 0)
        epi.noise = noise.data_ptr()
        epi.noise_stride = noise.shape[1]
        epi.noise_w = noise_w.data_ptr()
        epi.noise_b = noise_b.data_ptr()
    if residual is not None:
        assert is_cl(residual) and residual.shape == y.shape and residual.dtype == adt
        flags |= EPI_RESIDUAL
        epi.residual = residual.data_ptr()
        epi.res_scale = res_scale
    mask = None
    if want_mask and lrelu is True and conv_mask_supported(sh, 0, flags | EPI_MASK_OUT, precision):
        mask = torch.empty((sh[0], sh[9], sh[10], sh[4] // 8), dtype=torch.uint8, device=x.device)
        flags |= EPI_MASK_OUT
        epi.mask = mask.data_ptr()
    shp = _shape(*sh)
    ws, ws_bytes = _split_workspace(lib, shp, 0, precision, x)
    _check(lib.stylex_conv2d_fwd(_ptr(x), _ptr(wf), _ptr(y), shp, flags, ctypes.byref(epi), precision, _ptr(ws),
                                 ws_bytes, _stream()), "stylex_conv2d_fwd")
    return (y, mask) if want_mask else y


def conv2d_bwd_data(dy, w, x_shape, stride, pad, precision, in_scale=None, out_scale=None, packed=None, w_shape=None,
                    s2d_c=0, gate=None, gate_slope=0.2, gate_mask=None):
    lib = _ensure_device(dy)
    adt = act_dtype(precision)
    assert is_cl(dy) and dy.dtype == adt, (dy.dtype, adt)
    sh = conv_shape(x_shape, w_shape if packed is not None else w.shape, stride, pad)
    assert tuple(dy.shape) == (sh[0], sh[4], sh[9], sh[10]), (dy.shape, sh)
    wb = packed if packed is not None else pack_weight(w, False, True, precision)[1]
    dx = empty_cl(tuple(x_shape), dy, adt)
    epi = ConvEpilogue()
    epi.s2d_c = int(s2d_c)
    flags = 0
    in_scale, out_scale = _f32(in_scale), _f32(out_scale)
    if in_scale is not None:
        epi.in_scale = in_scale.data_ptr()
    if out_scale is not None:
        flags |= EPI_OSCALE
        epi.out_scale = out_scale.data_ptr()
    if gate_mask is not None and in_scale is None and out_scale is None and conv_mask_supported(sh, 1, EPI_GATE_MASK, precision):
        assert gate_mask.dtype == torch.uint8 and gate_mask.numel() * 8 == sh[0] * sh[1] * sh[2] * sh[3]
        flags |= EPI_GATE_MASK
        epi.mask = gate_mask.data_ptr()
        epi.res_scale = gate_slope
    elif gate is not None:
        assert is_cl(gate) and tuple(gate.shape) == tuple(x_shape) and gate.dtype == adt
        flags |= EPI_GATE
        epi.residual = gate.data_ptr()
        epi.res_scale = gate_slope
    else:
        assert gate_mask is None, "this launch cannot read a gate mask and no gate tensor was given"
    shp = _shape(*sh)
    ws, ws_bytes = _split_workspace(lib, shp, 1, precision, dy)
    _check(lib.stylex_conv2d_bwd_data(_ptr(dy), _ptr(wb), _ptr(dx), shp, flags, ctypes.byref(epi), precision,
                                      _ptr(ws), ws_bytes, _stream()), "stylex_conv2d_bwd_data")
    return dx


def pad_rgb8(x):
    lib = _ensure_device(x)
    assert x.dim() == 4 and x.shape[1] == 3 and x.dtype in (torch.float32, torch.bfloat16)
    b, _, h, w = x.shape
    y = _empty((b, h, w, 8), dtype=torch.bfloat16, device=x.device)
    shp = (ctypes.c_int64 * 3)(b, h, w)
    st = (ctypes.c_int64 * 4)(*x.stride())
    _check(lib.stylex_pad_rgb8(_ptr(x), _ptr(y), shp, st, int(x.dtype == torch.bfloat16), _stream()), "stylex_pad_rgb8")
    return y.permute(0, 3, 1, 2)


def _dense_f32(t):
    assert t.dtype == torch.float32 and t.is_contiguous(), "the frozen-classifier kernels take dense fp32 NCHW tensors"
# ... 293 lines not shown
    if nbytes < 0:
        raise StylexHipError("bad wgrad shape %r" % (sh,))
    ws = _empty(max(nbytes // 4, 1), dtype=torch.float32, device=x.device)
    x_scale, dy_scale = _f32(x_scale), _f32(dy_scale)
    if out_scale != 1.0 or accumulate_into is not None:
        acc = accumulate_into is not None
        dw = accumulate_into if acc else _empty(tuple(w_shape), dtype=torch.float32, device=x.device)
        raw = isinstance(dw, RawGrad)
        assert tuple(dw.shape) == tuple(w_shape) and (raw or (dw.dtype == torch.float32 and dw.is_contiguous()))
        db, written = None, ctypes.c_int(0)
        if want_bias_sum:
            db = accumulate_bias_into if (acc and accumulate_bias_into is not None) else None
            if acc and db is None:
                return conv2d_bwd_weight(x, dy, w_shape, stride, pad, precision, x_scale, dy_scale, s2d_c, False, out_scale,
                                         accumulate_into), None
            if db is None:
                db = _empty(w_shape[0], dtype=torch.float32, device=x.device)
        _check(lib.stylex_conv2d_bwd_weight_ex(_ptr(x), _ptr(dy), _ptr(dw), _ptr(db), ctypes.byref(written), _ptr(ws), nbytes, shp,
                                               _ptr(x_scale), _ptr(dy_scale), int(s2d_c), float(out_scale), int(acc), precision,
                                               _stream()), "stylex_conv2d_bwd_weight_ex")
        dw = None if raw else dw
        if want_bias_sum:
            if not written.value:
                return dw, None
            return dw, (True if isinstance(db, RawGrad) else db)
        return dw
    dw = _empty(tuple(w_shape), dtype=torch.float32, device=x.device)
    if want_bias_sum:
        db = _empty(w_shape[0], dtype=torch.float32, device=x.device)
        written = ctypes.c_int(0)
        _check(lib.stylex_conv2d_bwd_weight_bias(_ptr(x), _ptr(dy), _ptr(dw), _ptr(db), ctypes.byref(written), _ptr(ws), nbytes,
                                                 shp, _ptr(x_scale), _ptr(dy_scale), int(s2d_c), precision, _stream()),
               "stylex_conv2d_bwd_weight_bias")
        return dw, (db if written.value else None)
    _check(lib.stylex_conv2d_bwd_weight(_ptr(x), _ptr(dy), _ptr(dw), _ptr(ws), nbytes, shp, _ptr(x_scale),
                                        _ptr(dy_scale), int(s2d_c), precision, _stream()), "stylex_conv2d_bwd_weight")
    return dw


def _ew(fn_name, x, out_shape, in_shape_for_kernel):
    lib = _ensure_device(x)
    assert is_cl(x) and x.dtype in (torch.float32, torch.bfloat16)
    y = empty_cl(out_shape, x)
    b, c, h, w = in_shape_for_kernel
    _check(getattr(lib, fn_name)(_ptr(x), _ptr(y), _shape(b, h, w, c), _adt(x), _stream()), fn_name)
    return y


def upsample2x_fwd(x):
    b, c, h, w = x.shape
    return _ew("stylex_upsample2x_bilinear_fwd", x, (b, c, 2 * h, 2 * w), (b, c, h, w))


def upsample2x_bwd(dy):
    b, c, h2, w2 = dy.shape
    return _ew("stylex_upsample2x_bilinear_bwd", dy, (b, c, h2 // 2, w2 // 2), (b, c, h2 // 2, w2 // 2))


def rgb_up_blur_add_fwd(rgb, prev=None):
    lib = _ensure_device(rgb)
    assert is_cl(rgb) and rgb.dtype in (torch.float32, torch.bfloat16)
    assert prev is None or (is_cl(prev) and prev.dtype == rgb.dtype and prev.shape == rgb.shape)
    b, c, h, w = rgb.shape
    y = empty_cl((b, c, 2 * h, 2 * w), rgb)
    _check(lib.stylex_rgb_up_blur_add_fwd(_ptr(rgb), _ptr(prev), _ptr(y), _shape(b, h, w, c), _adt(rgb), _stream()),
           "stylex_rgb_up_blur_add_fwd")
    return y


def rgb_up_blur_add_bwd(dy):
    b, c, h2, w2 = dy.shape
    return _ew("stylex_rgb_up_blur_add_bwd", dy, (b, c, h2 // 2, w2 // 2), (b, c, h2 // 2, w2 // 2))


def blur3x3_fwd(x):
    return _ew("stylex_blur3x3_reflect_fwd", x, tuple(x.shape), tuple(x.shape))


def blur3x3_bwd(dy):
    return _ew("stylex_blur3x3_reflect_bwd", dy, tuple(dy.shape), tuple(dy.shape))


def blur3x3_s2d_fwd(x):
    lib = _ensure_device(x)
    assert is_cl(x)
    b, c, h, w = x.shape
    y = empty_cl((b, 4 * c, h // 2, w // 2), x)
    _check(lib.stylex_blur3x3_s2d_fwd(_ptr(x), _ptr(y), _shape(b, h, w, c), _adt(x), _stream()), "stylex_blur3x3_s2d_fwd")
    return y


def blur_mask_ok(shape, dtype):
    _, c, h, w = shape
    return dtype == torch.bfloat16 and c % 8 == 0 and h >= 8 and h % 2 == 0 and w % 2 == 0


def blur3x3_s2d_bwd(dy2, gate=None, slope=0.2, gate_mask=None):
    lib = _ensure_device(dy2)
    assert is_cl(dy2)
    b, c4, h2, w2 = dy2.shape
    dx = empty_cl((b, c4 // 4, 2 * h2, 2 * w2), dy2)
    shp = _shape(b, 2 * h2, 2 * w2, c4 // 4)
    if gate_mask is not None:
        assert gate_mask.dtype == torch.uint8 and gate_mask.numel() * 8 == dx.numel()
        _check(lib.stylex_blur3x3_s2d_bwd_gate_mask(_ptr(dy2), _ptr(gate_mask), float(slope), _ptr(dx), shp, _adt(dy2),
                                                    _stream()), "stylex_blur3x3_s2d_bwd_gate_mask")
# ... 170 lines not shown
    flat = not per_sample and b > 1
    if flat:
        nbytes = b * h * w * c * dy.element_size()
        h, b = b * h, 1
    shp = _shape(b, h, w, c)
    nch = lib.stylex_reduce_chunks(shp)
    if flat:
        nch = max(1, min(nch, max(64, -(-nbytes // (64 * 1024)))))
    partial = _empty((b, nch, c), dtype=torch.float32, device=dy.device)
    dx = empty_cl(tuple(dy.shape), dy) if want_dx else None
    _check(lib.stylex_act_bwd_reduce(_ptr(dy), _ptr(y), _ptr(dx), _ptr(partial), shp, nch, 2 if lrelu == "relu" else int(bool(lrelu)),
                                     float(scale), _adt(dy), _stream()), "stylex_act_bwd_reduce")
    return dx, ((partial.sum(dim=1) if per_sample else partial.sum(dim=(0, 1))) if want_sum else None)


def modconv_bwd_prep(gy, y, noise, noise_w, noise_b, lrelu, gz_scale=None):
    lib = _ensure_device(gy)
    assert is_cl(gy) and is_cl(y) and gy.dtype == y.dtype
    b, c, h, w = gy.shape
    shp = _shape(b, h, w, c)
    nch = lib.stylex_reduce_chunks(shp)
    partial = _empty((b, nch, 3, c), dtype=torch.float32, device=gy.device)
    gz = empty_cl(tuple(gy.shape), gy)
    ns = 0
    noise, noise_w, noise_b = _f32(noise), _f32(noise_w), _f32(noise_b)
    if noise is not None:
        ns = noise.shape[1]
    lr = 2 if lrelu == "relu" else int(bool(lrelu))
    if gz_scale is None:
        _check(lib.stylex_modconv_bwd_prep(_ptr(gy), _ptr(y), _ptr(noise), ns, _ptr(noise_w), _ptr(noise_b), _ptr(gz),
                                           _ptr(partial), shp, nch, lr, _adt(gy), _stream()), "stylex_modconv_bwd_prep")
    else:
        gz_scale = _f32(gz_scale)
        _check(lib.stylex_modconv_bwd_prep_scaled(_ptr(gy), _ptr(y), _ptr(noise), ns, _ptr(noise_w), _ptr(noise_b),
                                                  _ptr(gz_scale), _ptr(gz), _ptr(partial), shp, nch, lr, _adt(gy), _stream()),
               "stylex_modconv_bwd_prep_scaled")
    return gz, partial.sum(dim=1)


def scale_reduce(x, t, s, want_gx=True):
    lib = _ensure_device(x)
    assert is_cl(x) and is_cl(t) and x.dtype == t.dtype
    b, c, h, w = x.shape
    shp = _shape(b, h, w, c)
    nch = lib.stylex_reduce_chunks(shp)
    partial = _empty((b, nch, c), dtype=torch.float32, device=x.device)
    gx = empty_cl(tuple(x.shape), x) if want_gx else None
    s = _f32(s)
    _check(lib.stylex_scale_reduce(_ptr(x), _ptr(t), _ptr(s), _ptr(gx), _ptr(partial), shp, nch, _adt(x), _stream()),
           "stylex_scale_reduce")
    return gx, partial.sum(dim=1)


def torgb_ok(x):
    c = x.shape[1]
    if os.environ.get("STYLEX_TORGB", "1") == "0":
        return False
    return x.is_cuda and x.dtype == torch.bfloat16 and 8 <= c <= 512 and (c & (c - 1)) == 0


def torgb_fwd(x, s1, w):
    lib = _ensure_device(x)
    assert is_cl(x) and x.dtype == torch.bfloat16
    b, c, h, wd = x.shape
    y = empty_cl((b, 4, h, wd), x)
    s1, w = _f32(s1), _f32(w)
    _check(lib.stylex_torgb_fwd(_ptr(x), _ptr(s1), _ptr(w), _ptr(y), _shape(b, h, wd, c), _stream()), "stylex_torgb_fwd")
    return y


def torgb_bwd(x, gy, s1, w, want_gx=True):
    lib = _ensure_device(x)
    assert is_cl(x) and is_cl(gy) and gy.shape[1] == 4 and x.dtype == gy.dtype == torch.bfloat16
    b, c, h, wd = x.shape
    shp = _shape(b, h, wd, c)
    nch = lib.stylex_torgb_chunks(shp)
    partial = _empty((b, nch, 3, c), dtype=torch.float32, device=x.device)
    gx = empty_cl(tuple(x.shape), x) if want_gx else None
    s1, w = _f32(s1), _f32(w)
    _check(lib.stylex_torgb_bwd(_ptr(x), _ptr(gy), _ptr(s1), _ptr(w), _ptr(gx), _ptr(partial), shp, _stream()),
           "stylex_torgb_bwd")
    return gx, (partial.sum(dim=1) if nch > 1 else partial[:, 0])


KERNELS_SEEN = set()
_TIMING_ON = False


import contextlib as _contextlib
import threading as _threading

_TIMING_TLS = _threading.local()


def timing_paused():
    return getattr(_TIMING_TLS, "depth", 0) > 0


@_contextlib.contextmanager
def timing_pause():
    lib = load_library()
    _TIMING_TLS.depth = getattr(_TIMING_TLS, "depth", 0) + 1
    lib.stylex_timing_pause(1)
    try:
        yield
    finally:
# ... 161 lines not shown
```

### explaining-in-style-reproducibility-study_amd/stylex/networks.py

```python
import atexit
import math
from math import log2

import os

import torch
import torch.nn.functional as F
from torch import nn

import ops


def exists(v):
    return v is not None


_SIDE = {}
atexit.register(_SIDE.clear)


def _side_stream(t, which=0):
    import os

    if not t.is_cuda or os.environ.get("STYLEX_STREAMS", "1") == "0":
# ... 171 lines not shown
class Conv2DMod(nn.Module):
    def __init__(self, in_chan, out_chan, kernel, demod=True, stride=1, dilation=1, eps=1e-8, **kwargs):
        super().__init__()
        assert stride == 1 and dilation == 1, "only the configuration the reference uses is implemented"
        self.filters, self.demod, self.kernel = out_chan, demod, kernel
        self.stride, self.dilation, self.eps = stride, dilation, eps
        self.weight = nn.Parameter(torch.randn((out_chan, in_chan, kernel, kernel)))
        nn.init.kaiming_normal_(self.weight, a=0, mode="fan_in", nonlinearity="leaky_relu")

    def forward(self, x, y):
        return ops.modulated_conv2d(x, y, self.weight, demod=self.demod, eps=self.eps)


class RGBBlock(nn.Module):
    def __init__(self, latent_dim, input_channel, upsample, rgba=False):
        super().__init__()
        self.input_channel = input_channel
        self.to_style = nn.Linear(latent_dim, input_channel)
        self.conv = Conv2DMod(input_channel, 4 if rgba else 3, 1, demod=False)
        self.upsample = nn.Sequential(Upsample2x(), Blur()) if upsample else None

    def forward(self, x, prev_rgb, istyle, style=None, padded=False):
        style = self.to_style(istyle) if style is None else style
        if padded and not self.conv.demod:
            fused = ops.rgb_block(x, prev_rgb, style, self.conv.weight, exists(self.upsample))
            if fused is not None:
                return fused
        if exists(prev_rgb) and prev_rgb.shape[1] == 4 and self.conv.weight.shape[0] == 3:
            prev_rgb = prev_rgb[:, :3]
        x = self.conv(x, style)
        if exists(prev_rgb):
            x = x + prev_rgb
        if exists(self.upsample):
            x = self.upsample(x)
        return x


class GeneratorBlock(nn.Module):
    def __init__(self, latent_dim, input_channels, filters, upsample=True, upsample_rgb=True, rgba=False):
        super().__init__()
        self.input_channels, self.filters = input_channels, filters
        self.num_style_coords = input_channels + filters
        self.upsample = Upsample2x() if upsample else None
        self.to_style1 = nn.Linear(latent_dim, input_channels)
        self.to_noise1 = nn.Linear(1, filters)
        self.conv1 = Conv2DMod(input_channels, filters, 3)
        self.to_style2 = nn.Linear(latent_dim, filters)
        self.to_noise2 = nn.Linear(1, filters)
        self.conv2 = Conv2DMod(filters, filters, 3)
        self.activation = leaky_relu()
        self.to_rgb = RGBBlock(latent_dim, filters, upsample_rgb, rgba)

    def forward_main(self, x, istyle, inoise, styles=None):
        if exists(self.upsample):
            x = self.upsample(x)
        coords = None
        self._rgb_style = None
        if styles is None:
            fused = ops.style_affines(istyle, self.to_style1, self.to_style2, self.to_rgb.to_style, self.__dict__.setdefault("_aff_cache", {}))
            if fused is not None:
                style1, style2, self._rgb_style, coords = fused
            else:
                style1, style2 = self.to_style1(istyle), self.to_style2(istyle)
        else:
            style1, style2 = styles
        x = ops.modconv_noise_act(x, style1, self.conv1.weight, inoise, self.to_noise1.weight[:, 0],
                                  self.to_noise1.bias, demod=self.conv1.demod, eps=self.conv1.eps)
        x = ops.modconv_noise_act(x, style2, self.conv2.weight, inoise, self.to_noise2.weight[:, 0],
                                  self.to_noise2.bias, demod=self.conv2.demod, eps=self.conv2.eps)
        return x, (coords if coords is not None else torch.cat([style1, style2], dim=-1))

    def forward(self, x, prev_rgb, istyle, inoise):
        x, coords = self.forward_main(x, istyle, inoise)
        rgb = self.to_rgb(x, prev_rgb, istyle, style=self.__dict__.pop("_rgb_style", None))
        return x, rgb, coords


class DiscriminatorBlock(nn.Module):
    def __init__(self, input_channels, filters, downsample=True):
        super().__init__()
        self.conv_res = HipConv2d(input_channels, filters, 1, stride=(2 if downsample else 1))
        self.net = nn.Sequential(HipConv2d(input_channels, filters, 3, padding=1, act=True), _FusedAct(),
                                 HipConv2d(filters, filters, 3, padding=1, act=True), _FusedAct())
        self.downsample = nn.Sequential(Blur(), HipConv2d(filters, filters, 3, padding=1, stride=2)) if downsample else None

    def forward(self, x):
        fused = getattr(ops.impl(), "dblock", None)
        if fused is not None:
            out = fused(x, self.conv_res, self.net[0], self.net[2], self.downsample[1] if exists(self.downsample) else None)
            if out is not None:
                return out
        side = _side_stream(x)
        if side is None:
            res = self.conv_res(x)
            x = self.net(x)
        else:
            main = torch.cuda.current_stream()
            side.wait_stream(main)
            x.record_stream(side)
            with torch.cuda.stream(side):
                res = self.conv_res(x)
            x = self.net(x)
            main.wait_stream(side)
            res.record_stream(main)
        if exists(self.downsample):
            down = self.downsample[1]
            return ops.blur_down(x, down.weight, down.bias, res, 1 / math.sqrt(2))
        return ops.residual_merge(x, res)


def generator_filters(image_size, network_capacity, fmap_max):
    n = int(log2(image_size) - 1)
    f = [min(fmap_max, network_capacity * 2 ** (i + 1)) for i in range(n)][::-1]
    return [f[0]] + f


def discriminator_filters(image_size, network_capacity, fmap_max, transparent=False):
    n = int(log2(image_size) - 1)
# ... 75 lines not shown
```

### explaining-in-style-reproducibility-study_amd/stylex/ops.py

```python
import math

import os

import torch
from contextlib import nullcontext as _nullcontext
import torch.nn.functional as F

import hip_backend as hb

_PRECISION = hb.F32


_NAMES = {"fp32": hb.F32, "f32": hb.F32, "bf16": hb.BF16_ACT, "bf16_f32act": hb.BF16}


def set_precision(name):
    global _PRECISION
    _PRECISION = _NAMES[name]


def get_precision():
    return {hb.F32: "fp32", hb.BF16_ACT: "bf16", hb.BF16: "bf16_f32act"}[_PRECISION]


# ... 404 lines not shown
            gb = None
        return gx, gw, gb, (gz if has_res and ctx.needs_input_grad[3] else None), None, None, None, None


class _ConvBiasActDD(torch.autograd.Function):

    @staticmethod
    def forward(ctx, x, w, bias, residual, stride, pad, lrelu, res_scale, s2d=0):
        x = _cl(x)
        if residual is not None:
            residual = _cl(residual)
        y = _fwd(x, w, stride, pad, s2d, bias=bias, lrelu=lrelu, residual=residual, res_scale=res_scale)
        ctx.save_for_backward(x, w, y if lrelu else None)
        ctx.cfg = (stride, pad, lrelu, float(res_scale) if residual is not None else 1.0, bias is not None,
                   residual is not None, s2d)
        return y

    @staticmethod
    def backward(ctx, gy):
        x, w, y = ctx.saved_tensors
        stride, pad, lrelu, scale, has_bias, has_res, s2d = ctx.cfg
        gz = _BiasActBwd.apply(gy, y.detach()) if lrelu else gy
        if scale != 1.0:
            gz = gz * scale
        gx = gw = gb = None
        if ctx.needs_input_grad[0]:
            gx = _Dgrad.apply(gz, w, tuple(x.shape), stride, pad, s2d)
        if _want_param_grad(ctx, 1):
            gw = _Wgrad.apply(x, gz, tuple(w.shape), stride, pad, s2d)
        if has_bias and _want_param_grad(ctx, 2):
            gb = _channel_sum(gz) if (not torch.is_grad_enabled() and gz.is_cuda and hb.is_cl(gz)) else gz.sum(dim=(0, 2, 3), dtype=torch.float32)
        return gx, gw, gb, (gz if has_res and ctx.needs_input_grad[3] else None), None, None, None, None, None


_NAT_NOISE = {}
import atexit as _atexit

_atexit.register(_NAT_NOISE.clear)


def _natural_noise(inoise):
    hit = _NAT_NOISE.get("k")
    if (hit is not None and hit[0] is inoise and hit[1] == inoise._version
            and not (inoise.is_cuda and torch.cuda.is_current_stream_capturing())):
        return hit[2]
    nat = inoise[:, :, :, 0].transpose(1, 2).contiguous().float()
    _NAT_NOISE["k"] = (inoise, inoise._version, nat)
    return nat


class _ModConvFast(torch.autograd.Function):

    @staticmethod
    def forward(ctx, x, s1, d, w, noise, nw, nb, pad, lrelu, noise_nat=None):
        x = _cl(x)
        pre = _PRECISION == hb.BF16_ACT and s1 is not None and x.shape[2] * x.shape[3] <= 64 and x.shape[1] % 64 == 0
        ctx.pre = pre
        if pre:
            x_in, s_in = (x.float() * s1[:, :, None, None]).to(x.dtype).contiguous(memory_format=torch.channels_last), None
        else:
            x_in, s_in = x, s1
        if noise_nat is not None and noise_nat.shape[1] % 4 == 0:
            y = hb.conv2d_fwd(x_in, w, 1, pad, _PRECISION, in_scale=s_in, out_scale=d, noise=noise_nat, noise_w=nw,
                              noise_b=nb, lrelu=lrelu, noise_natural=True)
        else:
            y = hb.conv2d_fwd(x_in, w, 1, pad, _PRECISION, in_scale=s_in, out_scale=d, noise=noise, noise_w=nw, noise_b=nb,
                              lrelu=lrelu)
        ctx.save_for_backward(x, s1, d, w, noise, nw, nb, y if (lrelu or d is not None or noise is not None) else None)
        ctx.cfg = (pad, lrelu)
        return y

    @staticmethod
    @torch.autograd.function.once_differentiable
    def backward(ctx, gy):
        x, s1, d, w, noise, nw, nb, y = ctx.saved_tensors
        pad, lrelu = ctx.cfg
        gy = _cl(gy)
        gd = gnw = gnb = None
        folded = False
        if y is not None and _reducible(gy.shape[1]):
            fold = d is not None and _PRECISION != hb.F32 and os.environ.get("STYLEX_FOLD_D", "1") != "0"
            gz, sums = hb.modconv_bwd_prep(gy, y, noise, nw, nb, lrelu, gz_scale=d if fold else None)
            folded = fold
            if d is not None:
                gd = sums[:, 0] / d
            if noise is not None:
                gnw, gnb = sums[:, 1:3].sum(0)
        elif y is not None:
            raise hb.StylexHipError("fused modulated conv needs C_out % 4 == 0")
        else:
            gz = gy
        gx = gs1 = gw = None
        if ctx.needs_input_grad[0] or ctx.needs_input_grad[1]:
            if folded:
                t = hb.conv2d_bwd_data(gz, w, tuple(x.shape), 1, pad, _PRECISION)
            elif ctx.pre and d is not None:
                gzd = (gz.float() * d[:, :, None, None]).to(gz.dtype).contiguous(memory_format=torch.channels_last)
                t = hb.conv2d_bwd_data(gzd, w, tuple(x.shape), 1, pad, _PRECISION)
            else:
                t = hb.conv2d_bwd_data(gz, w, tuple(x.shape), 1, pad, _PRECISION, in_scale=d)
            if _reducible(x.shape[1]):
                gx, gs1 = hb.scale_reduce(x, t, s1, want_gx=ctx.needs_input_grad[0])
            else:
                gs1 = (x.float() * t.float()).sum(dim=(2, 3))
                gx = (t.float() * s1[:, :, None, None]).to(t.dtype)
        if ctx.needs_input_grad[3]:
            gw = hb.conv2d_bwd_weight(x, gz, tuple(w.shape), 1, pad, _PRECISION, x_scale=s1, dy_scale=None if folded else d)
        return gx, gs1, gd, gw, None, gnw, gnb, None, None, None


class _ToRGBFast(torch.autograd.Function):

    @staticmethod
    def forward(ctx, x, s1, w):
        x = _cl(x)
        ctx.save_for_backward(x, s1, w)
        return hb.torgb_fwd(x, s1, w)

    @staticmethod
    @torch.autograd.function.once_differentiable
    def backward(ctx, gy):
        x, s1, w = ctx.saved_tensors
        gx, t = hb.torgb_bwd(x, _cl(gy), s1, w, want_gx=ctx.needs_input_grad[0])
        gs1 = gw = None
        if ctx.needs_input_grad[1]:
            gs1 = (t * w.reshape(1, 3, -1).float()).sum(dim=1)
        if ctx.needs_input_grad[2]:
            gw = (t * s1.float()[:, None, :]).sum(dim=0).reshape(w.shape).to(w.dtype)
        return gx, gs1, gw


class _RGBTailFast(torch.autograd.Function):

    @staticmethod
    def forward(ctx, rgb, prev):
        return hb.rgb_up_blur_add_fwd(_cl(rgb), _cl(prev) if prev is not None else None)

    @staticmethod
    @torch.autograd.function.once_differentiable
    def backward(ctx, gy):
        g = hb.rgb_up_blur_add_bwd(_cl(gy))
        return g, (g if ctx.needs_input_grad[1] else None)


class _BlurS2D(torch.autograd.Function):

    @staticmethod
    def forward(ctx, x):
        return hb.blur3x3_s2d_fwd(_cl(x))

    @staticmethod
    def backward(ctx, gy2):
        return _BlurS2DBwd.apply(gy2)


class _BlurS2DBwd(torch.autograd.Function):
    @staticmethod
    def forward(ctx, gy2):
        return hb.blur3x3_s2d_bwd(_cl(gy2))

# ... 367 lines not shown
            x, stride = _Subsample2.apply(x), 1
        if not padded_out:
            fn = _ConvBiasActFast if fast_enabled() else _ConvBiasActDD
            return fn.apply(x, weight, bias, residual, stride, padding, lrelu, res_scale)
        y = _Conv.apply(x, weight, stride, padding)
        if padded_out:
            y = y[:, :n_out]
        if lrelu:
            assert residual is None
            return _BiasAct.apply(y, bias)
        if bias is not None:
            y = y + bias.view(1, -1, 1, 1)
        if residual is not None:
            y = (y + residual) * res_scale
        return y

    @staticmethod
    def modulated_conv2d(x, style, weight, demod=True, eps=1e-8, coeffs=None):
        x = _act(x)
        s1, d_pre = coeffs if coeffs is not None else mod_coeffs(style, weight, demod, eps)
        k = weight.shape[2]
        pad = (k - 1) // 2
        n_out = weight.shape[0]
        if fast_enabled() and n_out == 3 and k == 1 and not demod and hb.torgb_ok(x):
            return _ToRGBFast.apply(x, s1, weight)[:, :3]
        w_run = weight
        if n_out == 3:
            w_run = torch.cat([weight, weight.new_zeros(1, *weight.shape[1:])], dim=0)
        if fast_enabled() and w_run.shape[0] % 4 == 0:
            d = d_pre
            if demod and n_out == 3:
                d = torch.cat([d, d.new_ones(d.shape[0], 1)], dim=1)
            y = _ModConvFast.apply(x, s1, d, w_run, None, None, None, pad, False)
            return y[:, :3] if n_out == 3 else y
        y = _Conv.apply(x * s1[:, :, None, None], w_run, 1, pad)
        if n_out == 3:
            y = y[:, :3]
        if demod:
            y = y * d_pre[:, :, None, None]
        return y

    @staticmethod
    def modconv_noise_act(x, style, weight, inoise, noise_w, noise_b, demod=True, eps=1e-8, coeffs=None):
        x = _act(x)
        if fast_enabled() and weight.shape[0] % 4 == 0:
            s1, d = coeffs if coeffs is not None else mod_coeffs(style, weight, demod, eps)
            plane = inoise[:, :, :, 0]
            nat = _natural_noise(inoise) if (x.is_cuda and os.environ.get("STYLEX_NOISE_NAT", "1") != "0") else None
            return _ModConvFast.apply(x, s1, d, weight, plane, noise_w, noise_b, (weight.shape[2] - 1) // 2, True, nat)
        return HipOps.noise_act(HipOps.modulated_conv2d(x, style, weight, demod, eps, coeffs=coeffs), inoise, noise_w,
                                noise_b)

    @staticmethod
    def noise_act(x, inoise, noise_w, noise_b):
        h, w = x.shape[2], x.shape[3]
        plane = inoise[:, :h, :w, 0].transpose(1, 2)
        n = plane[:, None, :, :] * noise_w.view(1, -1, 1, 1) + noise_b.view(1, -1, 1, 1)
        return _BiasAct.apply(_act(x + n), None)

    @staticmethod
    def upsample2x(x):
        return _Up.apply(_act(x))

    @staticmethod
    def blur3x3(x):
        return _Blur.apply(_act(x))

    @staticmethod
    def blur_down(x, weight, bias, residual, res_scale):
        b, c, h, w = x.shape
        if (_PRECISION != hb.F32 and c % 64 == 0 and weight.shape[0] % 4 == 0 and h % 2 == 0
                and w % 2 == 0 and w // 2 >= 16 and h // 2 >= 16 and tuple(weight.shape[2:]) == (3, 3)):
            x2 = _BlurS2D.apply(_act(x))
            if fast_enabled():
                return _DownS2DFast.apply(x2, weight, bias, _act(residual), res_scale)
            return _ConvBiasActDD.apply(x2, weight, bias, _act(residual), 1, 1, False, res_scale, c)
        return HipOps.conv2d(HipOps.blur3x3(x), weight, bias, stride=2, padding=1, residual=residual,
                             res_scale=res_scale)

    @staticmethod
    def rgb_block(x, prev_rgb, style, weight, upsample):
        if not fast_enabled() or os.environ.get("STYLEX_RGB_TAIL", "1") == "0":
            return None
        x = _act(x)
        if tuple(weight.shape[2:]) != (1, 1) or weight.shape[0] != 3 or not hb.torgb_ok(x):
            return None
        if prev_rgb is not None and (prev_rgb.shape[1] != 4 or prev_rgb.dtype != x.dtype):
            return None
        rgb = _ToRGBFast.apply(x, style + 1, weight)
        if upsample:
            return _RGBTailFast.apply(rgb, prev_rgb)
        return rgb if prev_rgb is None else rgb + prev_rgb

    @staticmethod
    def residual_merge(x, res):
        return (x + res) * (1 / math.sqrt(2))

    @staticmethod
    def dblock(x, conv_res, conv1, conv2, down):
        if not fast_enabled() or os.environ.get("STYLEX_DBLOCK", "1") == "0":
            return None
        if conv1.weight.shape[0] % 4 != 0:
            return None
        return _DBlockFast.apply(x, conv_res.weight, conv_res.bias, conv1.weight, conv1.bias, conv2.weight, conv2.bias,
                                 down.weight if down is not None else None, down.bias if down is not None else None,
                                 down is not None)
# ... 322 lines not shown
```

### include/stylex_hip.h

```cpp
#ifndef STYLEX_HIP_H
#define STYLEX_HIP_H

#include <stdint.h>

#ifdef __cplusplus
extern "C" {
#endif

#define STYLEX_F32 0
#define STYLEX_BF16 1
#define STYLEX_BF16_ACT 2

#define STYLEX_EINVAL (-1)
#define STYLEX_EWORKSPACE (-2)

#define STYLEX_CONV_NSHAPE 11

#define STYLEX_EPI_BIAS 1
#define STYLEX_EPI_LRELU 2
#define STYLEX_EPI_OSCALE 4
#define STYLEX_EPI_NOISE 8
#define STYLEX_EPI_RESIDUAL 16
#define STYLEX_EPI_RELU 32
#define STYLEX_EPI_NOISE_NAT 128
#define STYLEX_EPI_MASK_OUT 256
#define STYLEX_EPI_GATE_MASK 512
#define STYLEX_EPI_GATE 64

int stylex_init(int device);
const char* stylex_version(void);

int stylex_pack_weight(const float* w_oihw, void* w_fwd, void* w_bwd, const int64_t* shape, int precision,
                       void* stream);

typedef struct {
    const float* in_scale;
    const float* bias;
    const float* out_scale;
    const float* noise;
    int64_t noise_stride;
    const float* noise_w;
    const float* noise_b;
    const void* residual;
    float res_scale;
    int32_t s2d_c;
    void* mask;
} stylex_conv_epilogue;

int stylex_conv_mask_supported(const int64_t* shape, int which, int flags, int precision);

int64_t stylex_conv2d_workspace_bytes(const int64_t* shape, int which, int precision);

int stylex_conv2d_fwd(const void* x, const void* w_fwd, void* y, const int64_t* shape, int flags,
                      const stylex_conv_epilogue* epi, int precision, void* workspace, int64_t workspace_bytes,
                      void* stream);

int stylex_conv2d_s2d_res_supported(const int64_t* shape, int64_t s2d_c, int64_t res_c);
int stylex_conv2d_s2d_res_fwd(const void* x_s2d, const void* w_fwd_s2d, const void* x_res, const void* w_res, const float* bias,
                              void* y, const int64_t* shape, int64_t s2d_c, int64_t res_c, float scale, void* stream);

int stylex_conv2d_bwd_data(const void* dy, const void* w_bwd, void* dx, const int64_t* shape, int flags,
                           const stylex_conv_epilogue* epi, int precision, void* workspace, int64_t workspace_bytes,
                           void* stream);

int64_t stylex_conv2d_bwd_weight_workspace_bytes(const int64_t* shape);
int stylex_conv2d_bwd_weight(const void* x, const void* dy, float* dw, void* workspace, int64_t workspace_bytes,
                             const int64_t* shape, const float* x_scale, const float* dy_scale, int s2d_c,
                             int precision, void* stream);
int stylex_conv2d_bwd_weight_bias(const void* x, const void* dy, float* dw, float* db, int* db_written, void* workspace,
                                  int64_t workspace_bytes, const int64_t* shape, const float* x_scale,
                                  const float* dy_scale, int s2d_c, int precision, void* stream);
int stylex_conv2d_bwd_weight_ex(const void* x, const void* dy, float* dw, float* db, int* db_written, void* workspace,
                                int64_t workspace_bytes, const int64_t* shape, const float* x_scale, const float* dy_scale,
                                int s2d_c, float out_scale, int accumulate, int precision, void* stream);

int stylex_upsample2x_bilinear_fwd(const void* x, void* y, const int64_t* shape, int act_dtype, void* stream);
int stylex_upsample2x_bilinear_bwd(const void* dy, void* dx, const int64_t* shape, int act_dtype, void* stream);

int stylex_blur3x3_reflect_fwd(const void* x, void* y, const int64_t* shape, int act_dtype, void* stream);
int stylex_blur3x3_reflect_bwd(const void* dy, void* dx, const int64_t* shape, int act_dtype, void* stream);

int stylex_rgb_up_blur_add_fwd(const void* rgb, const void* prev, void* out, const int64_t* shape, int act_dtype,
                               void* stream);
int stylex_rgb_up_blur_add_bwd(const void* dy, void* dx, const int64_t* shape, int act_dtype, void* stream);

int stylex_blur3x3_s2d_fwd(const void* x, void* y_s2d, const int64_t* shape, int act_dtype, void* stream);
int stylex_blur3x3_s2d_bwd(const void* dy_s2d, void* dx, const int64_t* shape, int act_dtype, void* stream);
int stylex_blur3x3_reflect_bwd_gate(const void* dy, const void* gate, float slope, void* dx, const int64_t* shape,
                                    int act_dtype, void* stream);
int stylex_blur3x3_s2d_bwd_gate(const void* dy_s2d, const void* gate, float slope, void* dx, const int64_t* shape,
                                int act_dtype, void* stream);
int stylex_blur3x3_s2d_bwd_gate_mask(const void* dy_s2d, const void* mask, float slope, void* dx, const int64_t* shape,
                                     int act_dtype, void* stream);
int stylex_add_at_even(const void* src, void* dst, const int64_t* shape, int act_dtype, void* stream);

int stylex_subsample2_fwd(const void* x, void* y, const int64_t* shape, int act_dtype, void* stream);
int stylex_subsample2_bwd(const void* dy, void* dx, const int64_t* shape, int act_dtype, void* stream);
int stylex_pack_weight_s2d(const float* w_oihw, void* w_fwd, void* w_bwd, const int64_t* shape, void* stream);
int stylex_fold_weight_grad_s2d(const float* dw_s2d, float* dw_oihw, const int64_t* shape, void* stream);
int stylex_conv2d_bwd_weight_s2d_supported(const int64_t* shape, int s2d_c, int precision);
int stylex_conv2d_bwd_weight_s2d(const void* x2, const void* dy, float* dw_oihw, void* workspace, int64_t workspace_bytes,
                                 const int64_t* shape, int s2d_c, float out_scale, int accumulate, int precision, void* stream);

int stylex_bias_act_fwd(const void* x, const float* bias, const float* noise, int64_t noise_stride,
                        const float* noise_w, const float* noise_b, void* y, const int64_t* shape, int act_dtype,
                        void* stream);
int stylex_bias_act_bwd(const void* dy, const void* y, void* dx, const int64_t* shape, int act_dtype, void* stream);

int stylex_rowwise_sumsq(const float* x, float* out, const int64_t* shape, void* stream);

int stylex_pad_rgb8(const void* x, void* y, const int64_t* shape_bhw, const int64_t* strides_bchw, int x_is_bf16, void* stream);

int stylex_affine_act_nchw_fwd(const float* x, const float* scale, const float* shift, const float* residual, float* y, int64_t B,
                               int64_t C, int64_t HW, int relu, void* stream);
int stylex_affine_act_nchw_bwd(const float* gy, const float* y, const float* scale, float* gx, float* gres, int64_t B, int64_t C,
                               int64_t HW, int relu, void* stream);
int stylex_affine_relu_maxpool_fwd(const float* x, const float* scale, const float* shift, float* y, unsigned char* idx, int64_t B,
                                   int64_t C, int64_t H, int64_t W, void* stream);
int stylex_affine_relu_maxpool_bwd(const float* gy, const unsigned char* idx, const float* scale, float* gx, int64_t B, int64_t C,
                                   int64_t H, int64_t W, void* stream);

int stylex_resize_norm_fwd(const float* x, float* y, const float* mean, const float* stdv, const int64_t* sh, const int64_t* strides,
                           void* stream);
int stylex_resize_norm_bwd(const float* gy, float* gx, const float* stdv, const int64_t* sh, void* stream);

int stylex_relu_gate_add(const void* a, const void* b, const void* y, void* out, int64_t numel, void* stream);
int stylex_nchw_f32_to_nhwc_bf16(const float* x, void* y, int64_t B, int64_t C, int64_t HW, int relu, void* stream);
int stylex_nhwc_bf16_to_nchw_f32(const void* g, const void* gate, float* gx, int64_t B, int64_t C, int64_t HW, void* stream);

int stylex_maxpool3s2_nhwc_fwd(const void* x, void* y, void* idx, const int64_t* sh, void* stream);
int stylex_maxpool3s2_nhwc_bwd(const void* gy, const void* idx, void* gx, const int64_t* sh, void* stream);

int stylex_conv_image_grad(const float* dy, const float* w, float* dx, const int64_t* sh, void* stream);

int stylex_lpips_tap_fwd(const float* f0, const float* f1, const float* lin, float* partial, float* r0, float* r1, int64_t B,
                         int64_t C, int64_t HW, int64_t partial_stride, void* stream);
int stylex_lpips_tap_bwd(const float* f0, const float* f1, const float* lin, const float* r0, const float* r1, const float* gout,
                         float* g0, float* g1, int64_t B, int64_t C, int64_t HW, void* stream);

int stylex_lpips_tap_nhwc_fwd(const void* f0, const void* f1, const float* lin, float* partial, float* r0, float* r1, int64_t B,
                              int64_t C, int64_t HW, int64_t partial_stride, void* stream);
int stylex_lpips_tap_nhwc_bwd(const void* f0, const void* f1, const float* lin, const float* r0, const float* r1, const float* gout,
                              void* g0, void* g1, int64_t B, int64_t C, int64_t HW, void* stream);

int stylex_weight_sumsq(const float* w, float* wsq, int64_t O, int64_t C, int64_t K, void* stream);
int stylex_modcoeff_fwd(const float* style, const float* wsq, float* s1, float* d, int64_t B, int64_t C, int64_t O,
                        float eps, void* stream);
int stylex_modcoeff_bwd(const float* gd, const float* d, const float* s1, const float* wsq, const float* w,
                        const float* gs1, float* gstyle, float* gw, int64_t B, int64_t C, int64_t O, int64_t K,
                        void* stream);

int stylex_reduce_chunks(const int64_t* shape);
int stylex_act_bwd_reduce(const void* dy, const void* y, void* dx, float* partial, const int64_t* shape, int nchunks,
                          int lrelu, float scale, int act_dtype, void* stream);
int stylex_modconv_bwd_prep(const void* gy, const void* y, const float* noise, int64_t noise_stride,
                            const float* noise_w, const float* noise_b, void* gz, float* partial,
                            const int64_t* shape, int nchunks, int lrelu, int act_dtype, void* stream);
int stylex_modconv_bwd_prep_scaled(const void* gy, const void* y, const float* noise, int64_t noise_stride,
                                   const float* noise_w, const float* noise_b, const float* gz_scale, void* gz,
                                   float* partial, const int64_t* shape, int nchunks, int lrelu, int act_dtype,
                                   void* stream);
int stylex_scale_reduce(const void* x, const void* t, const float* s, void* gx, float* partial, const int64_t* shape,
                        int nchunks, int act_dtype, void* stream);

int stylex_torgb_chunks(const int64_t* shape);
int stylex_torgb_fwd(const void* x, const float* s1, const float* w, void* y, const int64_t* shape, void* stream);
int stylex_torgb_bwd(const void* x, const void* gy, const float* s1, const float* w, void* gx, float* partial,
                     const int64_t* shape, void* stream);

int stylex_timing_enable(int on);
int stylex_timing_pause(int on);
int stylex_timing_report(int kernel_class, int64_t* launches, double* total_ms, double* total_flops,
                         double* total_bytes);
int stylex_timing_layers(int64_t* meta, double* vals, int64_t cap);
int stylex_timing_kernels(char* names, int64_t* meta, double* vals, int64_t cap);

#define STYLEX_ADAM_COPY_PACK 0
#define STYLEX_ADAM_COPY_PACK_S2D 1
#define STYLEX_ADAM_COPY_SUMSQ 2
typedef struct {
    float* p;
    const float* g;
    float* m;
    float* v;
    const float* step;
    int64_t numel;
    int32_t N, C, T, nvar;
    int64_t first_block;
    double lr, beta1, beta2, eps;
    struct {
        int32_t kind;
        float scale;
        void* a;
        void* b;
    } var[4];
} stylex_adam_tensor;
int64_t stylex_adam_pack_tensor_blocks(int64_t numel, int32_t N, int32_t C, int32_t T);
int stylex_adam_pack_step(const stylex_adam_tensor* descs_dev, const int32_t* block_map_dev, int64_t n_blocks, void* stream);

int stylex_hinge_fwd(const float* real, const float* fake, float* out, int64_t n, int mode, void* stream);
int stylex_hinge_bwd(const float* real, const float* fake, const float* gout, float* greal, float* gfake, int64_t n, int mode,
                     void* stream);
int stylex_pl_lengths_fwd(const float* g, float* len, const int64_t* shape, void* stream);
int stylex_pl_lengths_bwd(const float* g, const float* len, const float* glen, float* gg, const int64_t* shape, void* stream);
int stylex_kl_logits_fwd(const float* real, const float* fake, float* out, const int64_t* shape, void* stream);
int stylex_kl_logits_bwd(const float* real, const float* fake, const float* gout, float* greal, float* gfake, const int64_t* shape,
                         void* stream);
int64_t stylex_l1_mean_chunks(int64_t n);
int stylex_l1_mean_fwd(const void* a, const void* b, float* partial, float* out, int64_t n, int a_dtype, int b_dtype,
                       const int64_t* shape4, const int64_t* a_strides4, const int64_t* b_strides4, void* stream);
int stylex_l1_mean_bwd(const void* a, const void* b, const float* gout, void* ga, void* gb, int64_t n, int a_dtype, int b_dtype,
                       const int64_t* shape4, const int64_t* a_strides4, const int64_t* b_strides4, void* stream);

int stylex_linattn_chunks(const int64_t* shape);
int stylex_linattn_fwd(const void* q, const void* k, const void* v, const int64_t* strides, void* y, void* pre, float* context,
                       float* lse, float* workspace, const int64_t* shape, int act_dtype, void* stream);
// ... 18 lines not shown
```

Measured before the change: 999.0 images/sec.

## Fuse generator block upsample, modulation, and noise epilogues into conv kernels

Adds a modulated-conv epilogue mode to the halo-DMA and pipelined conv kernels. It applies the demod scale, the noise injection and leaky-ReLU, and can also write a copy pre-scaled by the next conv's style. The generator block then runs upsample+modulate as one kernel, and conv1 emits conv2's modulated input directly, skipping separate upsample, modulate and activation passes. A new backward fuses the scale-reduce with upsample. The cost is extra registers, LDS and many new shape and alignment guards.

```diff
diff --git a/explaining-in-style-reproducibility-study_amd/csrc/conv_halo_dma.hip b/explaining-in-style-reproducibility-study_amd/csrc/conv_halo_dma.hip
--- a/explaining-in-style-reproducibility-study_amd/csrc/conv_halo_dma.hip
+++ b/explaining-in-style-reproducibility-study_amd/csrc/conv_halo_dma.hip
@@ -69,7 +69,7 @@
 __device__ __forceinline__ int s2d_fwd_taps(int q) { return q == 0 ? 0x4 : q == 1 ? 0x43 : q == 2 ? 0x41 : 0x4310; }
 __device__ __forceinline__ int s2d_fwd_ntaps(int q) { return q == 0 ? 1 : q == 3 ? 4 : 2; }
 
-template <int TNJ, bool S2D = false>
+template <int TNJ, bool S2D = false, bool MOD = false>
 __global__ __launch_bounds__(256, TNJ == 4 ? 1 : 2) void conv3x3_halo_dma_kernel(ConvKParams p) {
     constexpr int BN = DmaCfg<TNJ>::BN, PIECES = DmaCfg<TNJ>::PIECES, NIT = DmaCfg<TNJ>::NIT, BUF = DmaCfg<TNJ>::BUF;
     extern __shared__ __attribute__((aligned(16))) char smem[];
@@ -280,6 +280,72 @@
                 b4[j][g] = ((p.flags & STYLEX_EPI_BIAS) && n < N) ? *reinterpret_cast<const float4*>(p.bias + n)
                                                                   : make_float4(0.f, 0.f, 0.f, 0.f);
             }
+        if (MOD) {
+            unsigned short* ynext = reinterpret_cast<unsigned short*>(p.y_next);
+            float4 d4[TNJ][4], w4[TNJ][4], c4[TNJ][4], s4[TNJ][4];
+#pragma unroll
+            for (int j = 0; j < TNJ; ++j)
+#pragma unroll
+                for (int g = 0; g < 4; ++g) {
+                    const int n = n0 + j * 32 + 8 * g + 4 * lh;
+                    const int nc = min(n, N - 4);
+                    d4[j][g] = *reinterpret_cast<const float4*>(p.out_scale + (long)b * N + nc);
+                    w4[j][g] = *reinterpret_cast<const float4*>(p.noise_w + nc);
+                    c4[j][g] = *reinterpret_cast<const float4*>(p.noise_b + nc);
+                    s4[j][g] = *reinterpret_cast<const float4*>((p.scale_next ? p.scale_next : p.out_scale) + (long)b * N + nc);
+                }
+#pragma unroll
+            for (int i = 0; i < 4; ++i) {
+                const int y = y0 + 4 * wave + i, x = x0 + lj;
+                const bool pix_ok = y < H && x < W;
+                const long obase = ((long)(b * H + y) * W + x) * N;
+                const float nz = pix_ok ? p.noise[((long)b * p.noise_stride + y) * p.noise_stride + x] : 0.f;
+#pragma unroll
+                for (int j = 0; j < TNJ; ++j) {
+                    unsigned P[4][2], Q[4][2];
+#pragma unroll
+                    for (int g = 0; g < 4; ++g) {
+                        float v0 = acc[i][j][4 * g + 0] * d4[j][g].x, v1 = acc[i][j][4 * g + 1] * d4[j][g].y;
+                        float v2 = acc[i][j][4 * g + 2] * d4[j][g].z, v3 = acc[i][j][4 * g + 3] * d4[j][g].w;
+                        v0 += nz * w4[j][g].x + c4[j][g].x;
+                        v1 += nz * w4[j][g].y + c4[j][g].y;
+                        v2 += nz * w4[j][g].z + c4[j][g].z;
+                        v3 += nz * w4[j][g].w + c4[j][g].w;
+                        v0 = v0 > 0.f ? v0 : 0.2f * v0;
+                        v1 = v1 > 0.f ? v1 : 0.2f * v1;
+                        v2 = v2 > 0.f ? v2 : 0.2f * v2;
+                        v3 = v3 > 0.f ? v3 : 0.2f * v3;
+                        const unsigned short h0 = to_bf16(v0), h1 = to_bf16(v1), h2 = to_bf16(v2), h3 = to_bf16(v3);
+                        P[g][0] = (unsigned)h0 | ((unsigned)h1 << 16);
+                        P[g][1] = (unsigned)h2 | ((unsigned)h3 << 16);
+                        Q[g][0] = (unsigned)to_bf16(__uint_as_float((unsigned)h0 << 16) * s4[j][g].x) |
+                                  ((unsigned)to_bf16(__uint_as_float((unsigned)h1 << 16) * s4[j][g].y) << 16);
+                        Q[g][1] = (unsigned)to_bf16(__uint_as_float((unsigned)h2 << 16) * s4[j][g].z) |
+                                  ((unsigned)to_bf16(__uint_as_float((unsigned)h3 << 16) * s4[j][g].w) << 16);
+                    }
+#pragma unroll
+                    for (int g = 0; g < 4; g += 2)
+#pragma unroll
+                        for (int h = 0; h < 2; ++h) {
+                            auto r = __builtin_amdgcn_permlane32_swap(P[g][h], P[g + 1][h], false, false);
+                            P[g][h] = r[0];
+                            P[g + 1][h] = r[1];
+                            auto r2 = __builtin_amdgcn_permlane32_swap(Q[g][h], Q[g + 1][h], false, false);
+                            Q[g][h] = r2[0];
+                            Q[g + 1][h] = r2[1];
+                        }
+#pragma unroll
+                    for (int q = 0; q < 2; ++q) {
+                        const int n = n0 + j * 32 + 16 * q + 8 * lh;
+                        if (pix_ok && n < N) {
+                            if (yout) *reinterpret_cast<uint4*>(yout + obase + n) = make_uint4(P[2 * q][0], P[2 * q][1], P[2 * q + 1][0], P[2 * q + 1][1]);
+                            if (ynext) *reinterpret_cast<uint4*>(ynext + obase + n) = make_uint4(Q[2 * q][0], Q[2 * q][1], Q[2 * q + 1][0], Q[2 * q + 1][1]);
+                        }
+                    }
+                }
+            }
+            return;
+        }
 #pragma unroll
         for (int i = 0; i < 4; ++i) {
             const int y = y0 + 4 * wave + i, x = x0 + lj;
@@ -353,19 +419,20 @@
 
 }
 
-template <int TNJ, bool S2D = false>
+template <int TNJ, bool S2D = false, bool MOD = false>
 static int launch_dma(const ConvKParams& p, hipStream_t s) {
     static bool attr_done = false;
     if (!attr_done) {
-        hipError_t e = hipFuncSetAttribute(reinterpret_cast<const void*>(conv3x3_halo_dma_kernel<TNJ, S2D>),
+        hipError_t e = hipFuncSetAttribute(reinterpret_cast<const void*>(conv3x3_halo_dma_kernel<TNJ, S2D, MOD>),
                                            hipFuncAttributeMaxDynamicSharedMemorySize, DmaCfg<TNJ>::SMEM_BYTES);
         if (e != hipSuccess) return (int)e;
         attr_done = true;
     }
     long tiles = (long)p.B * ((p.Wo + TW - 1) / TW) * ((p.Ho + TH - 1) / TH);
     long blocks = tiles * ((p.N + DmaCfg<TNJ>::BN - 1) / DmaCfg<TNJ>::BN);
-    stylex_note_kernel("conv3x3_halo_dma_kernel<%d, %s>", TNJ, S2D ? "true" : "false");
-    hipLaunchKernelGGL((conv3x3_halo_dma_kernel<TNJ, S2D>), dim3((unsigned)blocks), dim3(256), DmaCfg<TNJ>::SMEM_BYTES, s, p);
+    if (MOD) stylex_note_kernel("conv3x3_halo_dma_kernel<%d, %s, true>", TNJ, S2D ? "true" : "false");
+    else stylex_note_kernel("conv3x3_halo_dma_kernel<%d, %s>", TNJ, S2D ? "true" : "false");
+    hipLaunchKernelGGL((conv3x3_halo_dma_kernel<TNJ, S2D, MOD>), dim3((unsigned)blocks), dim3(256), DmaCfg<TNJ>::SMEM_BYTES, s, p);
     return (int)hipGetLastError();
 }
 
@@ -375,6 +442,20 @@
     static const bool on_s2d = !(getenv("STYLEX_HALO_DMA_S2D") && getenv("STYLEX_HALO_DMA_S2D")[0] == '0');
     if (!on) return STYLEX_NOT_APPLICABLE;
     if (!p.act_bf16 || p.a_scale) return STYLEX_NOT_APPLICABLE;
+    if ((p.flags & (STYLEX_EPI_OSCALE | STYLEX_EPI_NOISE)) || p.y_next) {
+        if (p.flags != (STYLEX_EPI_OSCALE | STYLEX_EPI_NOISE | STYLEX_EPI_NOISE_NAT | STYLEX_EPI_LRELU) || p.s2d_c || p.flip_taps ||
+            p.x2 || p.mask || p.gate_mask)
+            return STYLEX_NOT_APPLICABLE;
+        if (!p.out_scale || !p.noise || !p.noise_w || !p.noise_b || p.noise_stride < p.Ho || p.noise_stride < p.Wo) return STYLEX_NOT_APPLICABLE;
+        const void* quads[6] = {p.out_scale, p.noise_w, p.noise_b, p.scale_next, p.y, p.y_next};
+        for (const void* q : quads)
+            if (q && (reinterpret_cast<uintptr_t>(q) & 15)) return STYLEX_NOT_APPLICABLE;
+        if ((!p.y && !p.y_next) || (p.y_next && !p.scale_next)) return STYLEX_NOT_APPLICABLE;
+        if (p.N != 32 || p.Ck < 32 || p.Ck % 16 != 0 || p.Wo < 32 || p.Ho < 16) return STYLEX_NOT_APPLICABLE;
+        if ((reinterpret_cast<uintptr_t>(p.a) & 15) || (reinterpret_cast<uintptr_t>(p.w) & 15)) return STYLEX_NOT_APPLICABLE;
+        return p.dry ? 0 : launch_dma<1, false, true>(p, s);
+    }
+    if (!p.y) return STYLEX_NOT_APPLICABLE;
     if (p.flags & ~(STYLEX_EPI_BIAS | STYLEX_EPI_LRELU | STYLEX_EPI_RELU |
                     (p.s2d_c ? STYLEX_EPI_RESIDUAL : (STYLEX_EPI_GATE | STYLEX_EPI_GATE_MASK | STYLEX_EPI_MASK_OUT))))
         return STYLEX_NOT_APPLICABLE;
diff --git a/explaining-in-style-reproducibility-study_amd/csrc/conv_pipe.hip b/explaining-in-style-reproducibility-study_amd/csrc/conv_pipe.hip
--- a/explaining-in-style-reproducibility-study_amd/csrc/conv_pipe.hip
+++ b/explaining-in-style-reproducibility-study_amd/csrc/conv_pipe.hip
@@ -51,6 +51,8 @@
     static constexpr int BIAS_BASE = W_BASE + WS * W_STRIDE;
     static constexpr int DUMP_BASE = BIAS_BASE + 2048;
     static constexpr int SMEM = DUMP_BASE + 1024;
+    static constexpr int MOD_BASE = SMEM;
+    static constexpr int SMEM_MOD = SMEM + 8 * 1024;
     static constexpr int HP_MAX = (H_PIECES + 7) / 8;
     static constexpr int WP_MAX = (W_PIECES + 7) / 8;
     static constexpr int RG = TH / 4;
@@ -231,16 +233,99 @@
     const unsigned lane_off = (unsigned)(((4 * rg) * W + (lane & 7)) * N + nh * 64) * 2u +
                               (unsigned)(4 * ((lane >> 4) & 1) + 2 * ((lane >> 3) & 1) + (lane >> 5)) * 16u;
     const unsigned pixb8 = (unsigned)N * 16u;
+    auto xpose_store = [&](u32x4 (&R)[4], __amdgpu_buffer_rsrc_t rdst, unsigned soff, bool row_ok, int x0) {
+#pragma unroll
+            for (int j = 0; j < 2; ++j)
+#pragma unroll
+                for (int d = 0; d < 4; ++d) {
+                    const unsigned a0 = R[2 * j][d], a1 = R[2 * j + 1][d];
+                    R[2 * j][d] = (unsigned)__builtin_amdgcn_update_dpp((int)a0, (int)a1, 0x128, 0xF, 0xC, false);
+                    R[2 * j + 1][d] = (unsigned)__builtin_amdgcn_update_dpp((int)a1, (int)a0, 0x128, 0xF, 0x3, false);
+                }
+#pragma unroll
+            for (int q = 0; q < 2; ++q)
+#pragma unroll
+                for (int d = 0; d < 4; ++d) {
+                    auto r = __builtin_amdgcn_permlane16_swap(R[q][d], R[2 + q][d], false, false);
+                    R[q][d] = r[0];
+                    R[2 + q][d] = r[1];
+                }
+            if (!(PIPE_DBG & 1)) {
+#pragma unroll
+                for (int k = 0; k < 4; ++k) {
+                    const unsigned voff = (row_ok && x0 + 8 * k + (lane & 7) < W) ? lane_off : OOB;
+                    __builtin_amdgcn_raw_buffer_store_b128(R[k], rdst, voff, soff + k * pixb8, PIPE_STORE_AUX);
+                    asm volatile("s_nop 1" : "+v"(R[k]) : : "memory");
+                }
+            }
+    };
+    const __amdgpu_buffer_rsrc_t rnext = __builtin_amdgcn_make_buffer_rsrc(EPI == 3 ? p.y_next : p.y, 0, (int)bytes_y, 0x00020000);
     auto epilogue = [&](int b, int y0, int x0, int n0) {
         const int lh = lk;
         const int nb = n0 + nh * 64;
         const unsigned t_off = __builtin_amdgcn_readfirstlane((unsigned)((((long)(b * H + y0) * W + x0) * N + n0) * 2));
         const unsigned g_off = x0 + li < W ? (unsigned)(((4 * rg) * W + li) * N + nh * 64 + 8 * lh) * 2u : OOB;
+        float* const mv = reinterpret_cast<float*>(smem + Cfg::MOD_BASE + wave * 1024);
+        if (EPI == 3) {
+            mv[lane] = p.out_scale[(long)b * N + nb + lane];
+            mv[64 + lane] = p.noise_w[nb + lane];
+            mv[128 + lane] = p.noise_b[nb + lane];
+            mv[192 + lane] = p.scale_next ? p.scale_next[(long)b * N + nb + lane] : 1.f;
+            asm volatile("s_waitcnt lgkmcnt(0)" ::: "memory");
+        }
 #pragma unroll
         for (int i = 0; i < 4; ++i) {
             const bool row_ok = y0 + 4 * rg + i < H;
             const unsigned soff = t_off + i * rowb;
             u32x4 R[4];
+            if (EPI == 3) {
+                const int yy = y0 + 4 * rg + i, xx = x0 + li;
+                const float nz = (row_ok && xx < W) ? p.noise[((long)b * p.noise_stride + yy) * p.noise_stride + xx] : 0.f;
+                u32x4 R2[4];
+#pragma unroll
+                for (int j = 0; j < 2; ++j) {
+                    unsigned P[4][2], Q[4][2];
+#pragma unroll
+                    for (int g = 0; g < 4; ++g) {
+                        const int cl = j * 32 + 8 * g + 4 * lh;
+                        const float4 d4 = *reinterpret_cast<const float4*>(mv + cl), w4 = *reinterpret_cast<const float4*>(mv + 64 + cl);
+                        const float4 c4 = *reinterpret_cast<const float4*>(mv + 128 + cl), s4 = *reinterpret_cast<const float4*>(mv + 192 + cl);
+                        float v0 = acc[i][j][4 * g + 0] * d4.x, v1 = acc[i][j][4 * g + 1] * d4.y;
+                        float v2 = acc[i][j][4 * g + 2] * d4.z, v3 = acc[i][j][4 * g + 3] * d4.w;
+                        v0 += nz * w4.x + c4.x;
+                        v1 += nz * w4.y + c4.y;
+                        v2 += nz * w4.z + c4.z;
+                        v3 += nz * w4.w + c4.w;
+                        v0 = v0 > 0.f ? v0 : 0.2f * v0;
+                        v1 = v1 > 0.f ? v1 : 0.2f * v1;
+                        v2 = v2 > 0.f ? v2 : 0.2f * v2;
+                        v3 = v3 > 0.f ? v3 : 0.2f * v3;
+                        P[g][0] = pack2(v0, v1);
+                        P[g][1] = pack2(v2, v3);
+                        Q[g][0] = pack2(__uint_as_float(P[g][0] << 16) * s4.x, __uint_as_float(P[g][0] & 0xffff0000u) * s4.y);
+                        Q[g][1] = pack2(__uint_as_float(P[g][1] << 16) * s4.z, __uint_as_float(P[g][1] & 0xffff0000u) * s4.w);
+                    }
+#pragma unroll
+                    for (int g = 0; g < 4; g += 2)
+#pragma unroll
+                        for (int h = 0; h < 2; ++h) {
+                            auto r = __builtin_amdgcn_permlane32_swap(P[g][h], P[g + 1][h], false, false);
+                            P[g][h] = r[0];
+                            P[g + 1][h] = r[1];
+                            auto r2 = __builtin_amdgcn_permlane32_swap(Q[g][h], Q[g + 1][h], false, false);
+                            Q[g][h] = r2[0];
+                            Q[g + 1][h] = r2[1];
+                        }
+#pragma unroll
+                    for (int q = 0; q < 2; ++q) {
+                        R[2 * j + q] = u32x4{P[2 * q][0], P[2 * q][1], P[2 * q + 1][0], P[2 * q + 1][1]};
+                        R2[2 * j + q] = u32x4{Q[2 * q][0], Q[2 * q][1], Q[2 * q + 1][0], Q[2 * q + 1][1]};
+                    }
+                }
+                if (p.y) xpose_store(R, ry, soff, row_ok, x0);
+                if (p.y_next) xpose_store(R2, rnext, soff, row_ok, x0);
+                continue;
+            }
 #pragma unroll
             for (int j = 0; j < 2; ++j) {
                 u32x4 gv[2];
@@ -460,7 +545,7 @@
     static bool attr_done = false;
     if (!attr_done) {
         hipError_t e = hipFuncSetAttribute(reinterpret_cast<const void*>(conv3x3_pipe_kernel<NT, EPI>),
-                                           hipFuncAttributeMaxDynamicSharedMemorySize, Cfg::SMEM);
+                                           hipFuncAttributeMaxDynamicSharedMemorySize, EPI == 3 ? Cfg::SMEM_MOD : Cfg::SMEM);
         if (e != hipSuccess) return (int)e;
         attr_done = true;
     }
@@ -483,12 +568,13 @@
     pa.dbg = 0;
 #endif
     stylex_note_kernel("conv3x3_pipe_kernel<%d, %d>", NT, EPI);
-    hipLaunchKernelGGL((conv3x3_pipe_kernel<NT, EPI>), dim3((unsigned)g_num_cus), dim3(512), Cfg::SMEM, s, p, pa);
+    hipLaunchKernelGGL((conv3x3_pipe_kernel<NT, EPI>), dim3((unsigned)g_num_cus), dim3(512), EPI == 3 ? Cfg::SMEM_MOD : Cfg::SMEM, s, p, pa);
     return (int)hipGetLastError();
 }
 
 template <int NT>
 int launch_pipe_epi(const ConvKParams& p, hipStream_t s) {
+    if (p.flags & STYLEX_EPI_OSCALE) return launch_pipe<NT, 3>(p, s);
     if (p.flags & STYLEX_EPI_GATE) return launch_pipe<NT, 1>(p, s);
     if (p.flags & STYLEX_EPI_GATE_MASK) return launch_pipe<NT, 2>(p, s);
     return launch_pipe<NT, 0>(p, s);
@@ -500,7 +586,16 @@
     const char* env = getenv("STYLEX_CONV_PIPE");
     if (env && env[0] == '0') return STYLEX_NOT_APPLICABLE;
     if (!p.act_bf16 || p.a_scale || p.s2d_c) return STYLEX_NOT_APPLICABLE;
-    if (p.flags & ~(STYLEX_EPI_BIAS | STYLEX_EPI_LRELU | STYLEX_EPI_RELU | STYLEX_EPI_GATE | STYLEX_EPI_GATE_MASK | STYLEX_EPI_MASK_OUT))
+    constexpr int MOD_FLAGS = STYLEX_EPI_OSCALE | STYLEX_EPI_NOISE | STYLEX_EPI_NOISE_NAT | STYLEX_EPI_LRELU;
+    if ((p.flags & (STYLEX_EPI_OSCALE | STYLEX_EPI_NOISE)) || p.y_next) {
+        if (p.flags != MOD_FLAGS || p.flip_taps || !p.out_scale || !p.noise || !p.noise_w || !p.noise_b) return STYLEX_NOT_APPLICABLE;
+        if (p.noise_stride < p.Ho || p.noise_stride < p.Wo) return STYLEX_NOT_APPLICABLE;
+        if (p.y_next && (!p.scale_next || (reinterpret_cast<uintptr_t>(p.y_next) & 15))) return STYLEX_NOT_APPLICABLE;
+        if (!p.y && !p.y_next) return STYLEX_NOT_APPLICABLE;
+    } else if (!p.y) {
+        return STYLEX_NOT_APPLICABLE;
+    }
+    if (p.flags & ~(MOD_FLAGS | STYLEX_EPI_BIAS | STYLEX_EPI_RELU | STYLEX_EPI_GATE | STYLEX_EPI_GATE_MASK | STYLEX_EPI_MASK_OUT))
         return STYLEX_NOT_APPLICABLE;
     if ((p.flags & STYLEX_EPI_GATE) && (!p.residual || (reinterpret_cast<uintptr_t>(p.residual) & 15))) return STYLEX_NOT_APPLICABLE;
     if (p.Ck < 64 || p.Ck % 32 != 0 || p.N % 64 != 0 || p.N > 512 || p.Wo < 32 || p.Ho < 16) return STYLEX_NOT_APPLICABLE;
diff --git a/explaining-in-style-reproducibility-study_amd/csrc/elementwise.hip b/explaining-in-style-reproducibility-study_amd/csrc/elementwise.hip
--- a/explaining-in-style-reproducibility-study_amd/csrc/elementwise.hip
+++ b/explaining-in-style-reproducibility-study_amd/csrc/elementwise.hip
@@ -47,18 +47,7 @@
     }
 };
 
-__device__ __forceinline__ void up_rule(int o, int n, int& lo, int& hi, float& w_hi) {
-    int k = o >> 1;
-    if (o & 1) {
-        lo = k;
-        hi = min(k + 1, n - 1);
-        w_hi = 0.25f;
-    } else {
-        lo = max(k - 1, 0);
-        hi = k;
-        w_hi = 0.75f;
-    }
-}
+__device__ __forceinline__ void up_rule(int o, int n, int& lo, int& hi, float& w_hi) { stylex_up_rule(o, n, lo, hi, w_hi); }
 __device__ __forceinline__ float up_coef(int o, int i, int n) {
     int lo, hi;
     float wh;
@@ -108,6 +97,36 @@
     }
 }
 
+__global__ void upsample2x_mod_fwd_kernel(const void* __restrict__ x, const float* __restrict__ s, void* __restrict__ y,
+                                          int B, int H, int W, int C) {
+    typedef Vec<8> V8;
+    const int cv = C / 8;
+    const long total = (long)B * 2 * H * 2 * W * cv;
+    for (long i = blockIdx.x * (long)blockDim.x + threadIdx.x; i < total; i += (long)gridDim.x * blockDim.x) {
+        int cq, ow, oh, b;
+        const long pix = decomp_index(i, cv, (2 * W), (2 * H), cq, ow, oh, b);
+        const int c = cq * 8;
+        int hl, hh, wl, wh_;
+        float fh, fw;
+        up_rule(oh, H, hl, hh, fh);
+        up_rule(ow, W, wl, wh_, fw);
+        const long base = (long)b * H * W * C + c;
+        F8 acc = V8::zero(), r0 = V8::zero(), r1 = V8::zero();
+        V8::fma(r0, 1.f - fw, V8::ld(x, base + ((long)hl * W + wl) * C, 1));
+        V8::fma(r0, fw, V8::ld(x, base + ((long)hl * W + wh_) * C, 1));
+        V8::fma(r1, 1.f - fw, V8::ld(x, base + ((long)hh * W + wl) * C, 1));
+        V8::fma(r1, fw, V8::ld(x, base + ((long)hh * W + wh_) * C, 1));
+        V8::fma(acc, 1.f - fh, r0);
+        V8::fma(acc, fh, r1);
+        const float4 u0 = act_unpack4(act_pack4(acc.a)), u1 = act_unpack4(act_pack4(acc.b));
+        const float4 s0 = *reinterpret_cast<const float4*>(s + (long)b * C + c);
+        const float4 s1 = *reinterpret_cast<const float4*>(s + (long)b * C + c + 4);
+        V8::st(y, pix * C + c,
+               F8{make_float4(u0.x * s0.x, u0.y * s0.y, u0.z * s0.z, u0.w * s0.w),
+                  make_float4(u1.x * s1.x, u1.y * s1.y, u1.z * s1.z, u1.w * s1.w)}, 1);
+    }
+}
+
 template <int V>
 __global__ void upsample2x_bwd_kernel(const void* __restrict__ dy, void* __restrict__ dx, int B, int H, int W, int C, int bf) {
     const int cv = C / V;
@@ -540,6 +559,14 @@
     if (B <= 0 || H <= 0 || W <= 0 || C <= 0) return STYLEX_EINVAL;
     LAUNCH_EW(upsample2x_fwd_kernel, (long)B * 4 * H * W * C, x, y, x, y, B, H, W, C, bf);
 }
+int stylex_upsample2x_mod_fwd(const void* x, const float* scale, void* y, EW_ARGS) {
+    EW_UNPACK
+    if (!x || !scale || !y || B <= 0 || H <= 0 || W <= 0 || C <= 0) return STYLEX_EINVAL;
+    if (!bf || C % 8 != 0 || !vec_ok(C, x, y) || (reinterpret_cast<uintptr_t>(scale) & 15)) return STYLEX_EINVAL;
+    hipLaunchKernelGGL(upsample2x_mod_fwd_kernel, dim3(grid_for((long)B * 4 * H * W * C / 8)), dim3(256), 0, s, x, scale, y, B, H,
+                       W, C);
+    return (int)hipGetLastError();
+}
 int stylex_upsample2x_bilinear_bwd(const void* dy, void* dx, EW_ARGS) {
     EW_UNPACK
     if (B <= 0 || H <= 0 || W <= 0 || C <= 0) return STYLEX_EINVAL;
diff --git a/explaining-in-style-reproducibility-study_amd/csrc/fused_bwd.hip b/explaining-in-style-reproducibility-study_amd/csrc/fused_bwd.hip
--- a/explaining-in-style-reproducibility-study_amd/csrc/fused_bwd.hip
+++ b/explaining-in-style-reproducibility-study_amd/csrc/fused_bwd.hip
@@ -176,6 +176,47 @@
                           g.active && c < C);
 }
 
+__global__ __launch_bounds__(NT) void scale_reduce_up_kernel(const void* __restrict__ x_low, const void* __restrict__ t,
+                                                            const float* __restrict__ s, void* __restrict__ gx,
+                                                            float* __restrict__ partial, int H, int W, int C, int nchunks) {
+    extern __shared__ __attribute__((aligned(16))) float smem[];
+    const int W2 = 2 * W, HW2 = 4 * H * W;
+    Geo g = make_geo(HW2, C, nchunks);
+    Acc<1> a;
+    a.zero();
+    const int c = g.cv * 4;
+    if (g.active && c < C) {
+        float4 s4 = ldp4(s + (long)g.b * C + c);
+        const long base = (long)g.b * HW2;
+        const long lbase = (long)g.b * H * W * C + c;
+        for (long p = g.p_begin + g.prow; p < g.p_end; p += g.rpp) {
+            const long o = (base + p) * C + c;
+            const int pi = (int)p, oh = pi / W2, ow = pi - oh * W2;
+            int hl, hh, wl, wh;
+            float fh, fw;
+            stylex_up_rule(oh, H, hl, hh, fh);
+            stylex_up_rule(ow, W, wl, wh, fw);
+            const float4 p00 = ld4(x_low, lbase + ((long)hl * W + wl) * C, 1), p01 = ld4(x_low, lbase + ((long)hl * W + wh) * C, 1);
+            const float4 p10 = ld4(x_low, lbase + ((long)hh * W + wl) * C, 1), p11 = ld4(x_low, lbase + ((long)hh * W + wh) * C, 1);
+            float4 tv = ld4(t, o, 1);
+            const float gw = 1.f - fw, gh = 1.f - fh;
+            auto up1 = [&](float a00, float a01, float a10, float a11) -> float {
+                const float r0 = fmaf(fw, a01, fmaf(gw, a00, 0.f)), r1 = fmaf(fw, a11, fmaf(gw, a10, 0.f));
+                return fmaf(fh, r1, fmaf(gh, r0, 0.f));
+            };
+            const float4 xv = act_unpack4(act_pack4(make_float4(up1(p00.x, p01.x, p10.x, p11.x), up1(p00.y, p01.y, p10.y, p11.y),
+                                                                up1(p00.z, p01.z, p10.z, p11.z), up1(p00.w, p01.w, p10.w, p11.w))));
+            a.v[0].x += xv.x * tv.x; a.v[0].y += xv.y * tv.y; a.v[0].z += xv.z * tv.z; a.v[0].w += xv.w * tv.w;
+            if (gx) {
+                tv.x *= s4.x; tv.y *= s4.y; tv.z *= s4.z; tv.w *= s4.w;
+                st4(gx, o, tv, 1);
+            }
+        }
+    }
+    block_reduce_store<1>(a, smem, g.cv, g.prow, g.CV, g.rpp, C, partial + ((long)g.b * nchunks + blockIdx.x) * C,
+                          g.active && c < C);
+}
+
 inline size_t reduce_smem(int C, int K) {
     int CV = (C + 3) / 4;
     if (CV > NT) CV = NT;
@@ -253,4 +294,17 @@
     return (int)hipGetLastError();
 }
 
-}
+int stylex_scale_reduce_up(const void* x_low, const void* t, const float* s, void* gx, float* partial, const int64_t* sh,
+                           int nchunks, int act_dtype, void* stream) {
+    if (act_dtype != 1) return STYLEX_EINVAL;
+    if (!x_low || !t || !s || !partial || !ok_shape(sh, nchunks) || sh[1] * sh[2] * 4 >= (1l << 31)) return STYLEX_EINVAL;
+    if ((reinterpret_cast<uintptr_t>(x_low) & 7) || (reinterpret_cast<uintptr_t>(t) & 7) || (reinterpret_cast<uintptr_t>(gx) & 7) ||
+        (reinterpret_cast<uintptr_t>(s) & 15))
+        return STYLEX_EINVAL;
+    int C = (int)sh[3];
+    hipLaunchKernelGGL(scale_reduce_up_kernel, dim3(nchunks, (unsigned)sh[0]), dim3(NT), reduce_smem(C, 1),
+                       (hipStream_t)stream, x_low, t, s, gx, partial, (int)sh[1], (int)sh[2], C, nchunks);
+    return (int)hipGetLastError();
+}
+
+}
diff --git a/explaining-in-style-reproducibility-study_amd/csrc/stylex_capi.hip b/explaining-in-style-reproducibility-study_amd/csrc/stylex_capi.hip
--- a/explaining-in-style-reproducibility-study_amd/csrc/stylex_capi.hip
+++ b/explaining-in-style-reproducibility-study_amd/csrc/stylex_capi.hip
@@ -278,8 +278,10 @@
 int stylex_conv2d_fwd(const void* x, const void* w_fwd, void* y, const int64_t* sh, int flags,
                       const stylex_conv_epilogue* epi, int precision, void* workspace, int64_t workspace_bytes,
                       void* stream) {
-    if (!x || !w_fwd || !y || !conv_shape_ok(sh)) return STYLEX_EINVAL;
+    const bool to_next = epi && epi->y_next;
+    if (!x || !w_fwd || (!y && !to_next) || !conv_shape_ok(sh)) return STYLEX_EINVAL;
     if (precision != STYLEX_F32 && precision != STYLEX_BF16 && precision != STYLEX_BF16_ACT) return STYLEX_EINVAL;
+    if (to_next && (precision != STYLEX_BF16_ACT || !epi->scale_next)) return STYLEX_EINVAL;
     ConvKParams p;
     fwd_params(p, sh);
     p.a = (const float*)x;
@@ -299,6 +301,8 @@
         p.residual = (const float*)epi->residual;
         p.res_scale = epi->res_scale;
         p.s2d_c = (int)epi->s2d_c;
+        p.y_next = epi->y_next;
+        p.scale_next = epi->y_next ? epi->scale_next : nullptr;
     }
     if (flags & STYLEX_EPI_GATE_MASK) return STYLEX_EINVAL;
     if (flags & STYLEX_EPI_MASK_OUT) {
@@ -316,6 +320,12 @@
     if (p.s2d_c && (p.Ck != 4 * p.s2d_c || p.KH != 3 || p.stride != 1 || p.pad != 1 || p.s2d_c % 64)) return STYLEX_EINVAL;
     double flops = 2.0 * p.M * (double)p.N * p.Ck * p.KH * p.KW / (p.s2d_c ? 4.0 : 1.0);
     ScopedTimer tm(0, flops, conv_bytes(sh, p.act_bf16 ? STYLEX_BF16_ACT : precision, false), (hipStream_t)stream, sh, p.s2d_c);
+    if (to_next) {
+        if (p.KH != 3 || p.KW != 3 || p.stride != 1 || p.pad != 1 || p.Hi != p.Ho || p.Wi != p.Wo) return STYLEX_EINVAL;
+        int rc = stylex_launch_pipe(p, (hipStream_t)stream);
+        if (rc == STYLEX_NOT_APPLICABLE) rc = stylex_launch_halo_dma(p, (hipStream_t)stream);
+        return rc == STYLEX_NOT_APPLICABLE ? STYLEX_EINVAL : rc;
+    }
     return stylex_launch_igemm(p, precision, workspace, workspace_bytes, (hipStream_t)stream);
 }
 
diff --git a/explaining-in-style-reproducibility-study_amd/csrc/stylex_internal.h b/explaining-in-style-reproducibility-study_amd/csrc/stylex_internal.h
--- a/explaining-in-style-reproducibility-study_amd/csrc/stylex_internal.h
+++ b/explaining-in-style-reproducibility-study_amd/csrc/stylex_internal.h
@@ -41,6 +41,8 @@
     int c2;
     float wg_scale;
     int wg_accumulate;
+    void* y_next;
+    const float* scale_next;
 };
 
 int stylex_launch_igemm(ConvKParams p, int precision, void* workspace, int64_t workspace_bytes, hipStream_t s);
@@ -64,6 +66,18 @@
         m |= (__uint_as_float(w[d] & 0xffff0000u) > 0.f ? 1u : 0u) << (2 * d + 1);
     }
     return m;
+}
+__device__ __forceinline__ void stylex_up_rule(int o, int n, int& lo, int& hi, float& w_hi) {
+    const int k = o >> 1;
+    if (o & 1) {
+        lo = k;
+        hi = min(k + 1, n - 1);
+        w_hi = 0.25f;
+    } else {
+        lo = max(k - 1, 0);
+        hi = k;
+        w_hi = 0.75f;
+    }
 }
 #endif
 int stylex_launch_halo(const ConvKParams& p, hipStream_t s);
diff --git a/explaining-in-style-reproducibility-study_amd/stylex/hip_backend.py b/explaining-in-style-reproducibility-study_amd/stylex/hip_backend.py
--- a/explaining-in-style-reproducibility-study_amd/stylex/hip_backend.py
+++ b/explaining-in-style-reproducibility-study_amd/stylex/hip_backend.py
@@ -34,6 +34,8 @@
         ("res_scale", ctypes.c_float),
         ("s2d_c", ctypes.c_int32),
         ("mask", ctypes.c_void_p),
+        ("y_next", ctypes.c_void_p),
+        ("scale_next", ctypes.c_void_p),
     ]
 
 
@@ -71,6 +73,7 @@
                                                     ctypes.c_int, ctypes.c_float, ctypes.c_int, ctypes.c_int, ctypes.c_void_p]),
     "stylex_upsample2x_bilinear_fwd": (ctypes.c_int, [_c_f, _c_f, _i64p, ctypes.c_int, ctypes.c_void_p]),
     "stylex_upsample2x_bilinear_bwd": (ctypes.c_int, [_c_f, _c_f, _i64p, ctypes.c_int, ctypes.c_void_p]),
+    "stylex_upsample2x_mod_fwd": (ctypes.c_int, [_c_f, _c_f, _c_f, _i64p, ctypes.c_int, ctypes.c_void_p]),
     "stylex_rgb_up_blur_add_fwd": (ctypes.c_int, [_c_f, _c_f, _c_f, _i64p, ctypes.c_int, ctypes.c_void_p]),
     "stylex_rgb_up_blur_add_bwd": (ctypes.c_int, [_c_f, _c_f, _i64p, ctypes.c_int, ctypes.c_void_p]),
     "stylex_blur3x3_reflect_fwd": (ctypes.c_int, [_c_f, _c_f, _i64p, ctypes.c_int, ctypes.c_void_p]),
@@ -88,6 +91,8 @@
                                                       ctypes.c_int, ctypes.c_int, ctypes.c_int, ctypes.c_void_p]),
     "stylex_scale_reduce": (ctypes.c_int, [_c_f, _c_f, _c_f, _c_f, _c_f, _i64p, ctypes.c_int, ctypes.c_int,
                                            ctypes.c_void_p]),
+    "stylex_scale_reduce_up": (ctypes.c_int, [_c_f, _c_f, _c_f, _c_f, _c_f, _i64p, ctypes.c_int, ctypes.c_int,
+                                              ctypes.c_void_p]),
     "stylex_pad_rgb8": (ctypes.c_int, [_c_f, _c_f, _i64p, _i64p, ctypes.c_int, ctypes.c_void_p]),
     "stylex_affine_act_nchw_fwd": (ctypes.c_int, [_c_f, _c_f, _c_f, _c_f, _c_f, ctypes.c_int64, ctypes.c_int64, ctypes.c_int64,
                                                   ctypes.c_int, ctypes.c_void_p]),
@@ -788,17 +793,25 @@
 
 def conv2d_fwd(x, w, stride, pad, precision, bias=None, lrelu=False, in_scale=None, out_scale=None, noise=None,
                noise_w=None, noise_b=None, residual=None, res_scale=1.0, packed=None, w_shape=None, s2d_c=0,
-               noise_natural=False, want_mask=False):
+               noise_natural=False, want_mask=False, next_scale=None, want_y=True):
     lib = _ensure_device(x)
     adt = act_dtype(precision)
     assert is_cl(x) and x.dtype == adt, (x.dtype, adt)
     sh = conv_shape(x.shape, w_shape if packed is not None else w.shape, stride, pad)
     wf = packed if packed is not None else pack_weight(w, True, False, precision)[0]
-    y = empty_cl((sh[0], sh[4], sh[9], sh[10]), x, adt)
+    assert want_y or next_scale is not None
+    y = empty_cl((sh[0], sh[4], sh[9], sh[10]), x, adt) if want_y else None
     flags = 0
     epi = ConvEpilogue()
     epi.s2d_c = int(s2d_c)
     keep = []
+    y_next = None
+    if next_scale is not None:
+        next_scale = _f32(next_scale)
+        keep.append(next_scale)
+        y_next = empty_cl((sh[0], sh[4], sh[9], sh[10]), x, adt)
+        epi.y_next = y_next.data_ptr()
+        epi.scale_next = next_scale.data_ptr()
     if in_scale is not None:
         in_scale = _f32(in_scale)
         keep.append(in_scale)
@@ -824,7 +837,7 @@
         epi.noise_w = noise_w.data_ptr()
         epi.noise_b = noise_b.data_ptr()
     if residual is not None:
-        assert is_cl(residual) and residual.shape == y.shape and residual.dtype == adt
+        assert is_cl(residual) and y is not None and residual.shape == y.shape and residual.dtype == adt
         flags |= EPI_RESIDUAL
         epi.residual = residual.data_ptr()
         epi.res_scale = res_scale
@@ -837,6 +850,8 @@
     ws, ws_bytes = _split_workspace(lib, shp, 0, precision, x)
     _check(lib.stylex_conv2d_fwd(_ptr(x), _ptr(wf), _ptr(y), shp, flags, ctypes.byref(epi), precision, _ptr(ws),
                                  ws_bytes, _stream()), "stylex_conv2d_fwd")
+    if next_scale is not None:
+        return y, y_next
     return (y, mask) if want_mask else y
 
 
@@ -1236,6 +1251,17 @@
     return _ew("stylex_upsample2x_bilinear_fwd", x, (b, c, 2 * h, 2 * w), (b, c, h, w))
 
 
+def upsample2x_mod_fwd(x, s):
+    lib = _ensure_device(x)
+    assert is_cl(x) and x.dtype == torch.bfloat16
+    b, c, h, w = x.shape
+    y = empty_cl((b, c, 2 * h, 2 * w), x)
+    s = _f32(s)
+    _check(lib.stylex_upsample2x_mod_fwd(_ptr(x), _ptr(s), _ptr(y), _shape(b, h, w, c), _adt(x), _stream()),
+           "stylex_upsample2x_mod_fwd")
+    return y
+
+
 def upsample2x_bwd(dy):
     b, c, h2, w2 = dy.shape
     return _ew("stylex_upsample2x_bilinear_bwd", dy, (b, c, h2 // 2, w2 // 2), (b, c, h2 // 2, w2 // 2))
@@ -1512,6 +1538,20 @@
     return gx, partial.sum(dim=1)
 
 
+def scale_reduce_up(x_low, t, s, want_gx=True):
+    lib = _ensure_device(t)
+    assert is_cl(x_low) and is_cl(t) and x_low.dtype == t.dtype == torch.bfloat16
+    b, c, h, w = x_low.shape
+    assert tuple(t.shape) == (b, c, 2 * h, 2 * w)
+    nch = lib.stylex_reduce_chunks(_shape(b, 2 * h, 2 * w, c))
+    partial = _empty((b, nch, c), dtype=torch.float32, device=t.device)
+    gx = empty_cl(tuple(t.shape), t) if want_gx else None
+    s = _f32(s)
+    _check(lib.stylex_scale_reduce_up(_ptr(x_low), _ptr(t), _ptr(s), _ptr(gx), _ptr(partial), _shape(b, h, w, c), nch,
+                                      _adt(t), _stream()), "stylex_scale_reduce_up")
+    return gx, partial.sum(dim=1)
+
+
 def torgb_ok(x):
     c = x.shape[1]
     if os.environ.get("STYLEX_TORGB", "1") == "0":
diff --git a/explaining-in-style-reproducibility-study_amd/stylex/networks.py b/explaining-in-style-reproducibility-study_amd/stylex/networks.py
--- a/explaining-in-style-reproducibility-study_amd/stylex/networks.py
+++ b/explaining-in-style-reproducibility-study_amd/stylex/networks.py
@@ -247,8 +247,6 @@
         self.to_rgb = RGBBlock(latent_dim, filters, upsample_rgb, rgba)
 
     def forward_main(self, x, istyle, inoise, styles=None):
-        if exists(self.upsample):
-            x = self.upsample(x)
         coords = None
         self._rgb_style = None
         if styles is None:
@@ -259,6 +257,12 @@
                 style1, style2 = self.to_style1(istyle), self.to_style2(istyle)
         else:
             style1, style2 = styles
+        if exists(self.upsample):
+            fused_convs = getattr(ops.impl(), "gen_block_convs", None)
+            y = fused_convs(x, style1, style2, self.conv1, self.conv2, inoise, self.to_noise1, self.to_noise2) if fused_convs else None
+            if y is not None:
+                return y, (coords if coords is not None else torch.cat([style1, style2], dim=-1))
+            x = self.upsample(x)
         x = ops.modconv_noise_act(x, style1, self.conv1.weight, inoise, self.to_noise1.weight[:, 0],
                                   self.to_noise1.bias, demod=self.conv1.demod, eps=self.conv1.eps)
         x = ops.modconv_noise_act(x, style2, self.conv2.weight, inoise, self.to_noise2.weight[:, 0],
diff --git a/explaining-in-style-reproducibility-study_amd/stylex/ops.py b/explaining-in-style-reproducibility-study_amd/stylex/ops.py
--- a/explaining-in-style-reproducibility-study_amd/stylex/ops.py
+++ b/explaining-in-style-reproducibility-study_amd/stylex/ops.py
@@ -480,8 +480,15 @@
 class _ModConvFast(torch.autograd.Function):
 
     @staticmethod
-    def forward(ctx, x, s1, d, w, noise, nw, nb, pad, lrelu, noise_nat=None):
+    def forward(ctx, x, s1, d, w, noise, nw, nb, pad, lrelu, noise_nat=None, x_mod=None):
         x = _cl(x)
+        if x_mod is not None:
+            ctx.pre = False
+            y = hb.conv2d_fwd(x_mod, w, 1, pad, _PRECISION, out_scale=d, noise=noise_nat, noise_w=nw, noise_b=nb,
+                              lrelu=lrelu, noise_natural=True)
+            ctx.save_for_backward(x, s1, d, w, noise, nw, nb, y)
+            ctx.cfg = (pad, lrelu)
+            return y
         pre = _PRECISION == hb.BF16_ACT and s1 is not None and x.shape[2] * x.shape[3] <= 64 and x.shape[1] % 64 == 0
         ctx.pre = pre
         if pre:
@@ -534,6 +541,57 @@
                 gx = (t.float() * s1[:, :, None, None]).to(t.dtype)
         if ctx.needs_input_grad[3]:
             gw = hb.conv2d_bwd_weight(x, gz, tuple(w.shape), 1, pad, _PRECISION, x_scale=s1, dy_scale=None if folded else d)
+        return gx, gs1, gd, gw, None, gnw, gnb, None, None, None, None
+
+
+def prod_mod_enabled():
+    return os.environ.get("STYLEX_PROD_MOD", "1") != "0"
+
+
+def _dma_modconv_ok(b, c, n, h, w):
+    if os.environ.get("STYLEX_CONV_PIPE", "")[:1] == "0" or os.environ.get("STYLEX_HALO_DMA", "")[:1] == "0":
+        return False
+    if h < 32 or w < 32:
+        return False
+    if n % 64 == 0:
+        return c >= 64 and c % 32 == 0 and n <= 512 and b * h * w * max(c, n) * 2 < 2 ** 31
+    return n == 32 and c >= 32 and c % 16 == 0
+
+
+class _GenConv1Fast(torch.autograd.Function):
+
+    @staticmethod
+    def forward(ctx, x_low, s1, d, w, noise, nw, nb, noise_nat, s_next, want_y):
+        x_low = _cl(x_low)
+        ctx.set_materialize_grads(False)
+        xs = hb.upsample2x_mod_fwd(x_low, s1)
+        y, ym = hb.conv2d_fwd(xs, w, 1, 1, _PRECISION, out_scale=d, noise=noise_nat, noise_w=nw, noise_b=nb, lrelu=True,
+                              noise_natural=True, next_scale=s_next, want_y=want_y)
+        if not want_y:
+            return None, ym
+        ctx.save_for_backward(x_low, xs, s1, d, w, noise, nw, nb, y)
+        ctx.mark_non_differentiable(ym)
+        return y, ym
+
+    @staticmethod
+    @torch.autograd.function.once_differentiable
+    def backward(ctx, gy, _gym):
+        if gy is None:
+            return (None,) * 10
+        x_low, xs, s1, d, w, noise, nw, nb, y = ctx.saved_tensors
+        gy = _cl(gy)
+        fold = os.environ.get("STYLEX_FOLD_D", "1") != "0"
+        gz, sums = hb.modconv_bwd_prep(gy, y, noise, nw, nb, True, gz_scale=d if fold else None)
+        gd = sums[:, 0] / d
+        gnw, gnb = sums[:, 1:3].sum(0)
+        gx = gs1 = gw = None
+        if ctx.needs_input_grad[0] or ctx.needs_input_grad[1]:
+            t = hb.conv2d_bwd_data(gz, w, tuple(xs.shape), 1, 1, _PRECISION, in_scale=None if fold else d)
+            gx_up, gs1 = hb.scale_reduce_up(x_low, t, s1, want_gx=ctx.needs_input_grad[0])
+            if gx_up is not None:
+                gx = hb.upsample2x_bwd(gx_up)
+        if ctx.needs_input_grad[3]:
+            gw = hb.conv2d_bwd_weight(xs, gz, tuple(w.shape), 1, 1, _PRECISION, dy_scale=None if fold else d)
         return gx, gs1, gd, gw, None, gnw, gnb, None, None, None
 
 
@@ -1007,6 +1065,30 @@
                                 noise_b)
 
     @staticmethod
+    def gen_block_convs(x_low, style1, style2, conv1, conv2, inoise, noise1, noise2):
+        if not (_PRECISION == hb.BF16_ACT and fast_enabled() and x_low.is_cuda and prod_mod_enabled()
+                and os.environ.get("STYLEX_NOISE_NAT", "1") != "0" and conv1.demod and conv2.demod):
+            return None
+        w1, w2 = conv1.weight, conv2.weight
+        b, c, h, w = x_low.shape
+        n = w1.shape[0]
+        if (tuple(w1.shape[1:]) != (c, 3, 3) or tuple(w2.shape) != (n, n, 3, 3) or c % 8 != 0 or not _reducible(c)
+                or not _dma_modconv_ok(b, c, n, 2 * h, 2 * w) or not _dma_modconv_ok(b, n, n, 2 * h, 2 * w)):
+            return None
+        nat = _natural_noise(inoise)
+        if nat.shape[1] % 4 != 0 or nat.shape[1] < 2 * h or nat.shape[2] < 2 * w:
+            return None
+        s1, d1 = mod_coeffs(style1, w1, True, conv1.eps)
+        s2, d2 = mod_coeffs(style2, w2, True, conv2.eps)
+        plane = inoise[:, :, :, 0]
+        nw1, nb1, nw2, nb2 = noise1.weight[:, 0], noise1.bias, noise2.weight[:, 0], noise2.bias
+        y1, y1m = _GenConv1Fast.apply(_act(x_low), s1, d1, w1, plane, nw1, nb1, nat, s2.detach(), torch.is_grad_enabled())
+        if y1 is None:
+            return hb.conv2d_fwd(y1m, w2, 1, 1, _PRECISION, out_scale=d2, noise=nat, noise_w=nw2, noise_b=nb2, lrelu=True,
+                                 noise_natural=True)
+        return _ModConvFast.apply(y1, s2, d2, w2, plane, nw2, nb2, 1, True, nat, y1m)
+
+    @staticmethod
     def noise_act(x, inoise, noise_w, noise_b):
         h, w = x.shape[2], x.shape[3]
         plane = inoise[:, :h, :w, 0].transpose(1, 2)
diff --git a/include/stylex_hip.h b/include/stylex_hip.h
--- a/include/stylex_hip.h
+++ b/include/stylex_hip.h
@@ -45,6 +45,8 @@
     float res_scale;
     int32_t s2d_c;
     void* mask;
+    void* y_next;
+    const float* scale_next;
 } stylex_conv_epilogue;
 
 int stylex_conv_mask_supported(const int64_t* shape, int which, int flags, int precision);
@@ -76,6 +78,7 @@
 
 int stylex_upsample2x_bilinear_fwd(const void* x, void* y, const int64_t* shape, int act_dtype, void* stream);
 int stylex_upsample2x_bilinear_bwd(const void* dy, void* dx, const int64_t* shape, int act_dtype, void* stream);
+int stylex_upsample2x_mod_fwd(const void* x, const float* scale, void* y, const int64_t* shape, int act_dtype, void* stream);
 
 int stylex_blur3x3_reflect_fwd(const void* x, void* y, const int64_t* shape, int act_dtype, void* stream);
 int stylex_blur3x3_reflect_bwd(const void* dy, void* dx, const int64_t* shape, int act_dtype, void* stream);
@@ -162,6 +165,8 @@
                                    void* stream);
 int stylex_scale_reduce(const void* x, const void* t, const float* s, void* gx, float* partial, const int64_t* shape,
                         int nchunks, int act_dtype, void* stream);
+int stylex_scale_reduce_up(const void* x_low, const void* t, const float* s, void* gx, float* partial, const int64_t* shape,
+                           int nchunks, int act_dtype, void* stream);
 
 int stylex_torgb_chunks(const int64_t* shape);
 int stylex_torgb_fwd(const void* x, const float* s1, const float* w, void* y, const int64_t* shape, void* stream);
```

Measured after the change: 1009 images/sec (median of 5 runs). Within noise of the previous version (+1.0%).
